# at-cg/PHI

Measured on AMD Instinct MI355X. Metric: read Gbases/s scored (49-hap MHC graph stand-in synMHC-49); reads resident in HBM, parsing and H2D excluded, higher is better.
Workload: dtype u64

## Files before the change

### phi_amd/build.py

```python
import os
import subprocess
import sys

ROOT = os.path.dirname(os.path.dirname(os.path.abspath(__file__)))
CSRC = os.path.join(ROOT, "phi_amd", "csrc")
HIPCC = os.environ.get("HIPCC", "/opt/rocm/bin/hipcc")
ARCH = "gfx950"

HIP_SOURCES = ["sketch.hip", "sketch_pooled.hip", "sketch_win_fixed.hip", "table.hip", "anchors.hip", "contexts.hip", "dp.hip", "dp_events.hip", "phi_abi.hip", "dev_mem.hip", "read_batches.hip", "text_stream.hip", "text_park.hip", "set_graph.hip", "phi_solve.hip", "solve_dev.hip", "phi_comm.hip", "phi_ipc.hip", "reads_text.hip", "walk_text.hip", "edit.hip", "edit_path.hip", "inflate.hip", "gfa_text.hip", "chop.hip", "vcf.hip", "ladder.hip", "panel.hip", "panel_score.hip", "scan.hip", "bam.hip", "calls.hip"]
HIP_HEADERS = ["phi_dev.h", "phi_kernels.h", "phi_ctx.h", "phi_dp_flags.h", "phi_host_par.h", "phi_wave.h", "dp_steps.h", "solve_host.h", "reads_host.h", "bam_header.h", "sketch_dev.h", "sketch_phases.inc", "sketch_minima.inc", "sketch_rounds.inc", "edit_band.inc", os.path.join("host", "panel_choose.h"), os.path.join("..", "..", "include", "phi_amd.h")]


def _run(cmd, cwd=None):
    print("+", " ".join(cmd), flush=True)
    subprocess.check_call(cmd, cwd=cwd)


def _stale(target, deps):
    if not os.path.exists(target):
        return True
    t = os.path.getmtime(target)
    return any(os.path.getmtime(d) > t for d in deps if os.path.exists(d))


EXTRA_FLAGS = {"sketch_pooled.hip": ["-mllvm", "-disable-machine-licm"]}


def build_device(force=False):
    objdir = os.path.join(ROOT, "build", "obj")
    os.makedirs(objdir, exist_ok=True)
    hdrs = [os.path.join(CSRC, h) for h in HIP_HEADERS]
    objs = []
    for src in HIP_SOURCES:
        s = os.path.join(CSRC, src)
        o = os.path.join(objdir, src.replace(".hip", ".o"))
        if force or _stale(o, [s] + hdrs):
            _run([HIPCC, f"--offload-arch={ARCH}", "-O3", "-std=c++17", "-fPIC", "-Wall", "-Wno-unused-function"]
                 + EXTRA_FLAGS.get(src, []) + ["-c", s, "-o", o])
        objs.append(o)
    lib = os.path.join(ROOT, "phi_amd", "libphi_amd.so")
    if force or _stale(lib, objs):
        tmp = f"{lib}.{os.getpid()}.tmp"
        _run([HIPCC, f"--offload-arch={ARCH}", "-shared", "-fPIC", "-o", tmp] + objs + ["-ldl"])
        os.replace(tmp, lib)
    return lib


def build_host(force=False):
    hostdir = os.path.join(CSRC, "host")
    if not os.path.isdir(hostdir):
        return None
    _run(["make", "-C", hostdir] + (["-B"] if force else []))
    return os.path.join(ROOT, "phi_amd", "libphi_host.so")


def build_all(force=False):
    build_device(force)
    build_host(force)


if __name__ == "__main__":
    build_all(force="--force" in sys.argv)
```

### phi_amd/csrc/phi_abi.hip

```cpp
#include <stdarg.h>
#include <stdio.h>
#include <string.h>
#include <algorithm>
#include <future>
#include "phi_ctx.h"
#include "phi_dev.h"

int phi_fail(phi_ctx *c, int code, const char *fmt, ...)
{
    char buf[512];
    va_list ap;
    va_start(ap, fmt);
    vsnprintf(buf, sizeof buf, fmt, ap);
    va_end(ap);
    if (c) {
        std::lock_guard<std::mutex> g(c->err_mu);
        c->last_error = buf;
    }
    return code;
}

int phi_hip_check(phi_ctx *c, hipError_t e, const char *what)
{
    if (e == hipSuccess) return PHI_OK;
    const int code = (e == hipErrorOutOfMemory) ? PHI_ERR_NOMEM : PHI_ERR_DEVICE;
    return phi_fail(c, code, "%s: %s", what, hipGetErrorString(e));
}

extern "C" {

const char *phi_strerror(int status)
{
    switch (status) {
    case PHI_OK: return "ok";
    case PHI_ERR_INVALID: return "invalid argument";
    case PHI_ERR_NOMEM: return "out of memory";
    case PHI_ERR_DEVICE: return "HIP device error";
    case PHI_ERR_STATE: return "call order violated";
    case PHI_ERR_UNSUPPORTED: return "unsupported input";
    case PHI_ERR_WALK: return "walk does not follow the graph";
    case PHI_ERR_OVERFLOW: return "internal table overflow";
    default: return "unknown status";
    }
}

const char *phi_last_error(const phi_ctx *ctx) { return ctx ? ctx->last_error.c_str() : ""; }

int phi_ctx_create(int device_id, phi_ctx **out)
{
    if (!out) return PHI_ERR_INVALID;
    *out = nullptr;
    PhiStageTimer tm("ctx_create");
    int n_dev = 0;
    if (hipGetDeviceCount(&n_dev) != hipSuccess || n_dev <= 0) return PHI_ERR_DEVICE;
    tm.lap("runtime start (hipInit)");
    if (device_id < 0 || device_id >= n_dev) return PHI_ERR_INVALID;
    if (hipSetDevice(device_id) != hipSuccess) return PHI_ERR_DEVICE;
    phi_ctx *c = new (std::nothrow) phi_ctx();
    if (!c) return PHI_ERR_NOMEM;
    c->device = device_id;
    std::future<hipError_t> aux = std::async(std::launch::async, [c, device_id]() {
        hipError_t e = hipSetDevice(device_id);
        if (e == hipSuccess) e = hipStreamCreateWithFlags(&c->aux_stream, hipStreamNonBlocking);
        if (e != hipSuccess) return e;
        void *d = nullptr;
        std::vector<char> h((size_t)1 << 20, 0);
        if (hipMalloc(&d, h.size()) == hipSuccess) {
            (void)phi_dev_poison(d, h.size());
            (void)hipMemcpyAsync(d, h.data(), h.size(), hipMemcpyHostToDevice, c->aux_stream);
            (void)hipMemcpyAsync(h.data(), d, h.size(), hipMemcpyDeviceToHost, c->aux_stream);
            (void)hipMemcpyAsync(d, h.data(), 64, hipMemcpyHostToDevice, c->aux_stream);
            (void)hipMemcpyAsync(h.data(), d, 64, hipMemcpyDeviceToHost, c->aux_stream);
            (void)hipMemsetAsync(d, 0, 4096, c->aux_stream);
            (void)hipStreamSynchronize(c->aux_stream);
            (void)hipFree(d);
        }
        return hipSuccess;
    });
    auto bail = [&](int code) {
        if (aux.valid()) (void)aux.get();
        if (c->own_stream) (void)hipStreamDestroy(c->own_stream);
        if (c->aux_stream) (void)hipStreamDestroy(c->aux_stream);
        phi_dev_free(c->d_scalars); phi_dev_free(c->d_stripes); phi_dev_free(c->alt.stripes);
        delete c;
        return code;
    };
    if (hipStreamCreateWithFlags(&c->own_stream, hipStreamNonBlocking) != hipSuccess) return bail(PHI_ERR_DEVICE);
    c->stream = c->own_stream;
    tm.lap("stream");
    if (phi_dev_ensure(c, c->d_scalars, S_N * 8) || hipMemsetAsync(c->d_scalars.p, 0, S_N * 8, c->stream) != hipSuccess ||
        phi_dev_ensure(c, c->d_stripes, 2 * STRIPE_BYTES) || hipMemsetAsync(c->d_stripes.p, 0, 2 * STRIPE_BYTES, c->stream) != hipSuccess ||
        phi_dev_ensure(c, c->alt.stripes, 2 * STRIPE_BYTES) || hipMemsetAsync(c->alt.stripes.p, 0, 2 * STRIPE_BYTES, c->stream) != hipSuccess)
        return bail(PHI_ERR_DEVICE);
    if (tm.on && getenv("PHI_TIMING_UNITS")) {
        (void)hipStreamSynchronize(c->stream); tm.lap("  scalars");
        phi_warm_sketch(c->stream); (void)hipStreamSynchronize(c->stream); tm.lap("  code object: sketch");
        phi_warm_table(c->stream); (void)hipStreamSynchronize(c->stream); tm.lap("  code object: table");
        phi_warm_anchors(c->stream); (void)hipStreamSynchronize(c->stream); tm.lap("  code object: anchors");
        phi_warm_contexts(c->stream); (void)hipStreamSynchronize(c->stream); tm.lap("  code object: contexts");
        phi_warm_dp(c->stream); (void)hipStreamSynchronize(c->stream); tm.lap("  code object: dp");
        phi_warm_dp_events(c->stream); (void)hipStreamSynchronize(c->stream); tm.lap("  code object: dp_events");
        phi_warm_solve_dev(c->stream); (void)hipStreamSynchronize(c->stream); tm.lap("  code object: solve_dev");
        phi_warm_reads_text(c->stream); (void)hipStreamSynchronize(c->stream); tm.lap("  code object: reads_text");
        phi_warm_scan(c->stream); (void)hipStreamSynchronize(c->stream); tm.lap("  code object: scan");
    }
    phi_warm_sketch(c->stream); phi_warm_table(c->stream); phi_warm_anchors(c->stream); phi_warm_contexts(c->stream);
    phi_warm_dp(c->stream); phi_warm_dp_events(c->stream); phi_warm_solve_dev(c->stream); phi_warm_reads_text(c->stream);
    phi_warm_walk_text(c->stream); phi_warm_scan(c->stream);
    if (hipStreamSynchronize(c->stream) != hipSuccess) return bail(PHI_ERR_DEVICE);
    tm.lap("scalars + code objects");
    if (aux.get() != hipSuccess) { c->aux_stream = nullptr; return bail(PHI_ERR_DEVICE); }
    c->last_error.clear();
    tm.lap("wait for the second stream + first host copies");
    *out = c;
    return PHI_OK;
}

void phi_ctx_destroy(phi_ctx *c)
{
    if (c && c->pin_future.valid()) c->pin_future.wait();
    if (c && c->dp_alloc_future.valid()) (void)c->dp_alloc_future.get();
    if (c && c->h_pin) { (void)hipSetDevice(c->device); (void)hipHostFree(c->h_pin); c->h_pin = nullptr; }
    if (c) { (void)hipSetDevice(c->device); stage_release(c); }
    if (!c) return;
    (void)phi_comm_destroy(c);
    (void)phi_ipc_destroy(c);
    (void)hipSetDevice(c->device);
    (void)hipStreamSynchronize(c->stream);
    phi_ladder_drop(c);
    DevBuf *all[] = {&c->d_anchors, &c->d_cov_all, &c->d_cov_w, &c->d_slots, &c->d_slots2, &c->d_segs, &c->d_ctr, &c->d_vmax, &c->d_lane_walk, &c->d_walk_lane, &c->d_coff, &c->d_blk_ncls, &c->d_rownew, &c->d_blk_bad, &c->d_seg_lo, &c->d_seg_row, &c->d_seg_S, &c->wtext.d_text, &c->panel.d_full, &c->scout.d_scores, &c->d_sel_off, &c->d_sel_tri, &c->d_blk_lo, &c->d_blk_ev, &c->d_blk_S, &c->d_row_out, &c->d_rowend, &c->d_blk_keys, &c->d_blk_carry, &c->d_cov, &c->d_cov2, &c->d_stepdiff, &c->alt.hit, &c->hit_extra[0], &c->hit_extra[1], &c->alt.stripes, &c->spset.d_sp_cnt, &c->rlog.d_novlog, &c->rlog.d_novcnt, &c->rlog.d_ovlist, &c->d_vlen, &c->d_ent_cls, &c->d_cls_rep, &c->d_cls_left, &c->d_cls_mult, &c->d_cls_base, &c->d_cls_rec_off, &c->d_rec_cls, &c->d_rec_rel, &c->d_u_replist, &c->d_adj_off, &c->d_adj, &c->d_topo_rank, &c->d_cnt_edge, &c->d_walk_err, &c->d_sa_cnt, &c->d_sa_cur, &c->d_sa_off, &c->d_sa_idx, &c->d_seq, &c->d_seq_off, &c->d_walk_vtx, &c->d_walk_off, &c->d_topo, &c->d_in_off,
                     &c->d_in_src, &c->d_e_out, &c->d_st_rec, &c->d_st_mask, &c->d_in_packed, &c->d_word, &c->d_wwords, &c->d_wbad,
                     &c->d_wascii, &c->d_wstarts, &c->d_rec_hash, &c->d_rec_pos, &c->d_rec_slot,
                     &c->d_rec_e0, &c->d_rec_e1, &c->d_u_keys, &c->d_u_rep, &c->d_u_uid, &c->d_rt, &c->d_in_s, &c->d_last_walk, &c->d_rowdiag, &c->d_wpre, &c->d_hit, &c->spset.d_sp_keys, &c->d_rbases,
                     &c->d_roff, &c->rlog.d_roff_made, &c->d_peer_send, &c->spset.d_export, &c->d_scalars, &c->d_stripes, &c->d_blk_cnt,
                     &c->d_blk_off, &c->d_flags, &c->d_flags2, &c->d_list, &c->d_list2, &c->d_list3, &c->d_walk_last, &c->d_m_rec, &c->d_m_group,
                     &c->d_g_keys, &c->d_g_rep, &c->d_g_cnt, &c->d_slot_maxcnt, &c->d_slot_multi, &c->d_a_e1,
                     &c->d_g_off, &c->d_g_span, &c->d_a_weight, &c->d_dmax, &c->d_bstart, &c->d_k_rec, &c->d_k_in, &c->d_cvtx, &c->d_ev_e, &c->d_ev_off, &c->d_ev,
                     &c->d_off_end, &c->d_off_start, &c->d_scan_blk, &c->d_scan_blk64, &c->d_scan_blkoff, &c->d_top,
                     &c->d_ent};
    phi_pool_flush(c->device);
    phi_pool_bypass(true);
    struct Bypass { ~Bypass() { phi_pool_bypass(false); } } bypass_guard;
    for (DevBuf *b : all) phi_dev_free(*b);
    for (auto &pr : c->prof_events) { (void)hipEventDestroy(pr.first); (void)hipEventDestroy(pr.second); }
    if (c->h_err) (void)hipHostFree(c->h_err);
    {
        auto &T = c->text;
        for (int i = 0; i < 2; i++) { phi_dev_free(T.text[i]); phi_dev_free(T.bases[i]); phi_dev_free(T.roff[i]); }
        phi_dev_free(T.tile_cnt); phi_dev_free(T.ls); phi_dev_free(T.pre); phi_dev_free(T.blk); phi_dev_free(T.sum);
        if (T.h_sum) (void)hipHostFree(T.h_sum);
        if (T.ev_copy) (void)hipEventDestroy(T.ev_copy);
    }
    phi_bam_drop(c);
    (void)hipStreamDestroy(c->own_stream);
    (void)hipStreamDestroy(c->aux_stream);
    delete c;
}

int phi_set_stream(phi_ctx *c, void *hip_stream)
{
    if (!c) return PHI_ERR_INVALID;
    HIPCHK(hipStreamSynchronize(c->stream));
    c->stream = hip_stream ? (hipStream_t)hip_stream : c->own_stream;
    return PHI_OK;
}

int phi_set_params(phi_ctx *c, int32_t k, int32_t w, float threshold, int32_t recombination, uint32_t flags)
{
    if (!c) return PHI_ERR_INVALID;
    if (c->have_graph) return phi_fail(c, PHI_ERR_STATE, "phi_set_params must precede phi_set_graph");
    if (k < 1 || k > PHI_MAX_K) return phi_fail(c, PHI_ERR_INVALID, "k=%d outside [1,%d]", k, PHI_MAX_K);
    if (w < 1 || w > PHI_MAX_W) return phi_fail(c, PHI_ERR_INVALID, "w=%d outside [1,%d]", w, PHI_MAX_W);
    if (recombination < 0) return phi_fail(c, PHI_ERR_INVALID, "recombination penalty must be >= 0");
    c->k = k; c->w = w; c->threshold = threshold; c->recombination = recombination; c->flags = flags;
    return PHI_OK;
}

}

int sketch_records(phi_ctx *c, const uint64_t *words, const unsigned long long *starts, int64_t n_bases,
                   int32_t k, int32_t w, const uint8_t *ascii_if_bad, DevBuf &out_hash, DevBuf &out_pos,
                   int64_t *n_out)
{
    *n_out = 0;
    const int64_t nb = phi_sketch_num_blocks(n_bases);
    if (nb == 0) return PHI_OK;
    PHICHK(phi_dev_ensure(c, c->d_blk_cnt, (size_t)nb * 4));
    PHICHK(phi_dev_ensure(c, c->d_blk_off, (size_t)(nb + 1) * 8));
    PhiSketchArgs A{};
    A.words = words; A.starts = starts; A.n_bases = n_bases; A.k = k; A.w = w;
    A.ascii = ascii_if_bad; A.allslow = ascii_if_bad ? 1 : 0; A.badbits = nullptr;
    A.block_cnt = c->d_blk_cnt.as<int32_t>();
    A.err = (uint32_t *)scalar(c, S_ERR);
    if (A.allslow) phi_launch_sketch_bytes(c->stream, PHI_MODE_COUNT, A, nullptr);
    else phi_launch_sketch(c->stream, PHI_MODE_COUNT, A);
    PHICHK(phi_scan(c, c->d_blk_cnt.as<int32_t>(), nb, c->d_blk_off.as<int64_t>()));
    int64_t total = 0;
    HIPCHK(hipMemcpyAsync(&total, c->d_blk_off.as<int64_t>() + nb, 8, hipMemcpyDeviceToHost, c->stream));
    HIPCHK(hipStreamSynchronize(c->stream));
    PHICHK(phi_dev_ensure(c, out_hash, (size_t)std::max<int64_t>(total, 1) * 8));
    PHICHK(phi_dev_ensure(c, out_pos, (size_t)std::max<int64_t>(total, 1) * 8));
    A.block_off = c->d_blk_off.as<int64_t>();
    A.out_hash = out_hash.as<uint64_t>();
    A.out_pos = out_pos.as<int64_t>();
    if (A.allslow) phi_launch_sketch_bytes(c->stream, PHI_MODE_WRITE, A, nullptr);
    else phi_launch_sketch(c->stream, PHI_MODE_WRITE, A);
    HIPCHK(hipGetLastError());
    *n_out = total;
    return PHI_OK;
}

extern "C" {

int phi_set_solve_budget(phi_ctx *c, int64_t max_dp_runs)
{
    if (!c) return PHI_ERR_INVALID;
    c->solve_budget = max_dp_runs > 0x7FFFFFFF ? 0x7FFFFFFF : max_dp_runs;
    c->solved = false;
    return PHI_OK;
}

int phi_solve(phi_ctx *c, phi_result *out)
{
    if (!c || !out) return PHI_ERR_INVALID;
    if (!c->have_graph) return phi_fail(c, PHI_ERR_STATE, "phi_solve before phi_set_graph");
    PHICHK(phi_refuse_scout(c, "phi_solve"));
    HIPCHK(hipSetDevice(c->device));
    const int rc = phi_solve_impl(c);
    phi_pool_flush(c->device);
    if (rc) return rc;
    *out = c->result;
    return PHI_OK;
}

int phi_path_sequence(phi_ctx *c, char *buf, int64_t cap)
{
    if (!c || (!buf && cap > 0)) return PHI_ERR_INVALID;
    PHICHK(phi_refuse_scout(c, "phi_path_sequence"));
    if (!c->solved) return phi_fail(c, PHI_ERR_STATE, "phi_path_sequence before phi_solve");
    if (cap < c->result.hap_len) return phi_fail(c, PHI_ERR_INVALID, "buffer too small: need %lld bytes", (long long)c->result.hap_len);
    const int64_t np = (int64_t)c->h_path_vtx.size();
    std::vector<int64_t> at((size_t)np + 1, 0);
    for (int64_t i = 0; i < np; i++) { const int32_t v = c->h_path_vtx[(size_t)i]; at[(size_t)i + 1] = at[(size_t)i] + (c->h_seq_off[v + 1] - c->h_seq_off[v]); }
    phi_parallel_chunks(np, 1 << 15, [&](int64_t lo, int64_t hi, int) {
        for (int64_t i = lo; i < hi; i++) {
            const int32_t v = c->h_path_vtx[(size_t)i];
            memcpy(buf + at[(size_t)i], c->h_seq.data() + c->h_seq_off[v], (size_t)(at[(size_t)i + 1] - at[(size_t)i]));
        }
    });
    return PHI_OK;
}

int phi_sketch(phi_ctx *c, const char *bases, const int64_t *seq_off, int64_t n_seq, int32_t k, int32_t w,
               uint64_t *out_hash, int64_t *out_pos, int32_t *out_seq, int64_t cap, int64_t *n_out)
{
    if (!c || !n_out || n_seq < 0 || (n_seq > 0 && !seq_off)) return PHI_ERR_INVALID;
    if (k < 1 || k > PHI_MAX_K || w < 1 || w > PHI_MAX_W) return phi_fail(c, PHI_ERR_INVALID, "k or w out of range");
    *n_out = 0;
    if (n_seq == 0) return PHI_OK;
    for (int64_t r = 0; r < n_seq; r++)
        if (seq_off[r + 1] < seq_off[r]) return phi_fail(c, PHI_ERR_INVALID, "seq_off not monotone");
    const int64_t n_bases = seq_off[n_seq] - seq_off[0];
    if (n_bases == 0) return PHI_OK;
    if (!bases) return PHI_ERR_INVALID;
    HIPCHK(hipSetDevice(c->device));
    HIPCHK(hipStreamSynchronize(c->stream));
    DevBuf dB, dO, dW, dS, dH, dP;
    int rc = PHI_OK;
    std::vector<int64_t> off(seq_off, seq_off + n_seq + 1);
    for (auto &o : off) o -= seq_off[0];
    do {
        if ((rc = phi_dev_ensure(c, dB, (size_t)n_bases + 64))) break;
        if ((rc = phi_dev_ensure(c, dO, (size_t)(n_seq + 1) * 8))) break;
        const int64_t n_words = (n_bases + 31) / 32;
        if ((rc = phi_dev_ensure(c, dW, (size_t)(n_words + 2) * 8))) break;
        const size_t n_sw = (size_t)(n_bases / 64 + 2);
        if ((rc = phi_dev_ensure(c, dS, n_sw * 8))) break;
        if ((rc = phi_hip_check(c, hipMemcpyAsync(dB.p, bases + seq_off[0], (size_t)n_bases, hipMemcpyHostToDevice, c->stream), "H2D bases"))) break;
        if ((rc = phi_hip_check(c, hipMemcpyAsync(dO.p, off.data(), (size_t)(n_seq + 1) * 8, hipMemcpyHostToDevice, c->stream), "H2D offsets"))) break;
        if ((rc = phi_hip_check(c, hipMemsetAsync(dW.as<uint64_t>() + n_words, 0, 16, c->stream), "memset"))) break;
        if ((rc = phi_hip_check(c, hipMemsetAsync(dS.p, 0, n_sw * 8, c->stream), "memset"))) break;
        if ((rc = phi_hip_check(c, hipMemsetAsync(scalar(c, S_NBAD), 0, 8, c->stream), "memset"))) break;
        phi_launch_mark_starts(c->stream, dO.as<int64_t>(), n_seq, dS.as<unsigned long long>());
        phi_launch_pack_ascii(c->stream, dB.as<uint8_t>(), n_bases, dW.as<uint64_t>(), n_words, nullptr,
                              (unsigned long long *)scalar(c, S_NBAD));
        if ((rc = phi_hip_check(c, hipStreamSynchronize(c->stream), "sync"))) break;
// ... 210 lines not shown
```

### phi_amd/csrc/phi_ctx.h

```cpp
#pragma once
#include <stdint.h>
#include <stdarg.h>
#include <stdio.h>
#include <stdlib.h>
#include <algorithm>
#include <atomic>
#include <chrono>
#include <future>
#include <mutex>
#include <string>
#include <thread>
#include <vector>
#include <hip/hip_runtime.h>
#include "../../include/phi_amd.h"
#include "phi_kernels.h"
#include "phi_host_par.h"
#include "solve_host.h"
#include "reads_host.h"

struct DevBuf {
    void *p = nullptr;
    size_t cap = 0;
    uint32_t gen = 0;
    template <class T> T *as() const { return reinterpret_cast<T *>(p); }
};

template <class T> struct PhiRawBuf {
    T *p = nullptr;
    size_t n = 0;
    PhiRawBuf() = default;
    PhiRawBuf(const PhiRawBuf &) = delete;
    PhiRawBuf &operator=(const PhiRawBuf &) = delete;
    ~PhiRawBuf() { free(p); }
    bool resize(size_t m)
    {
        free(p);
        p = m ? static_cast<T *>(malloc(m * sizeof(T))) : nullptr;
        n = p ? m : 0;
        return m == 0 || p != nullptr;
    }
    size_t size() const { return n; }
    T *data() const { return p; }
    T &operator[](size_t i) const { return p[i]; }
};

struct PhiComm;
struct PhiIpc;
#define PHI_HIT_RING 4
struct PhiPeers;

struct phi_ctx {
    int device = 0;
    PhiComm *comm = nullptr;
    PhiPeers *peers = nullptr;
    int peer_rank = 0;
    PhiIpc *ipc = nullptr;
    hipStream_t own_stream = nullptr, stream = nullptr;
    hipStream_t aux_stream = nullptr;
    std::string last_error;
    std::mutex err_mu;

    int32_t k = 31, w = 25, recombination = 100;
    float threshold = 1.0f;
    uint32_t flags = PHI_FLAG_QCLP | PHI_FLAG_MIXED;
    int64_t solve_budget = 4096;

    bool have_graph = false;
    int32_t n_vtx = 0, n_walks = 0;
    std::vector<char> h_seq;
    std::vector<int64_t> h_seq_off, h_adj_off, h_walk_off, h_walk_base;
    std::vector<int32_t> h_adj, h_topo_rank, h_topo;
    PhiRawBuf<int32_t> h_walk_vtx;
    int64_t n_entries = 0, walk_bases = 0;

#define WT_TILE 4096
    struct PhiWalkText {
        bool ready = false;
        int32_t n_walks = 0;
        std::vector<int64_t> tile0, t_len;
        std::vector<int32_t> ends;
        DevBuf d_text;
    } wtext;
    bool walks_on_device = false;
    int64_t walks_on_device_n = 0;
    struct PhiChop {
        bool on = false;
        std::vector<int32_t> first;
        phi_chop_info info{};
    } chop;
    struct PhiPanel {
        bool on = false;
        std::vector<int32_t> origin;
        std::vector<int32_t> kept;
        phi_panel_info info{};
        DevBuf d_full;
        std::vector<int64_t> full_off;
    } panel;
    struct PhiScout {
        bool on = false;
        DevBuf d_scores;
        int32_t n_blocks = 0;
    } scout;
    struct PhiVcf {
        bool have = false;
        phi_vcf_info info{};
    } vcf;

    DevBuf d_seq, d_seq_off, d_walk_vtx, d_walk_off, d_topo, d_in_off, d_in_src;
    DevBuf d_e_out, d_st_rec, d_st_mask, d_in_packed;
    int dp_nw = 1;
    DevBuf d_wwords, d_wstarts, d_wbad, d_wascii;
    DevBuf d_vlen;
    DevBuf d_ent_cls;
    DevBuf d_cls_rep, d_cls_left, d_cls_mult, d_cls_base, d_cls_rec_off;
    int64_t n_cls = 0, cls_bases = 0;
    double index_gpu_ms = 0.0;
    DevBuf d_rec_hash, d_rec_pos, d_rec_cls, d_rec_rel, d_rec_slot, d_rec_e0, d_rec_e1;
    int64_t n_rec = 0;
    DevBuf d_u_keys, d_u_rep, d_u_uid, d_u_replist;
    DevBuf d_rt;
    uint64_t rt_buckets = 0, rt_mask = 0;
    void *h_stage[2] = {nullptr, nullptr};
    hipEvent_t stage_ev[2] = {nullptr, nullptr};
    DevBuf d_wpre;
    DevBuf d_rowdiag;
    DevBuf d_in_s, d_last_walk;
    int64_t n_unique = 0;
    uint64_t u_cap = 0;
    DevBuf d_hit;
    DevBuf hit_extra[PHI_HIT_RING - 2];
    int hit_n = 2, hit_idx = 0;

    struct PhiSpectrumSet {
        DevBuf d_sp_keys;
        uint64_t sp_cap = 0;
        DevBuf d_sp_cnt;
        DevBuf d_export;
        int64_t sp_set_gen = -1;
        int64_t sp_gen = 0;
        void new_generation() { sp_gen++; }
        void new_graph() { sp_set_gen = -1; }
    } spset;
    struct PhiReadLog {
        DevBuf d_novlog, d_novcnt;
        int32_t nov_shift = 6;
        int64_t log_chunks = 0, log_done = 0;
        int64_t logged_done = 0;
        int64_t last_log_chunks = 0;
        DevBuf d_ovlist;
        int64_t ov_cap = 0, ov_done = 0, ov_bound = 0;
        bool async_batches = false;
        bool next_flag_zeroed = false;
        DevBuf d_roff_made;
        void flushed() { log_chunks = log_done = 0; ov_done = 0; ov_bound = 0; }
        void new_generation() { flushed(); logged_done = 0; last_log_chunks = 0; next_flag_zeroed = false; }
    } rlog;
    int64_t reads_bases = 0, reads_count = 0;
    int64_t spectrum_override = -1;
    DevBuf d_rbases, d_roff, d_peer_send;
    DevBuf d_scalars;
    DevBuf d_stripes;
    struct PhiReadBufs {
        DevBuf hit, stripes;
        bool needs_clean = false;
    } alt;

    uint32_t *h_err = nullptr;
    struct PhiTextStream {
        bool active = false, irregular = false, started = false, detached = false;
        bool carry_stale = false;
        int mode = 0;
        int64_t fed = 0, taken = 0;
        uint32_t carry_cap = 0, chunk_cap = 0, line_cap = 0;
        DevBuf text[2], bases[2], roff[2], tile_cnt, ls, pre, blk, sum;
        int slot = 0;
        uint32_t carry_len = 0, carry_at = 0;
        std::vector<char> h_carry;
        PhiTextSummary *h_sum = nullptr;
        hipEvent_t ev_copy = nullptr;
        int last_slot = -1;
        int64_t last_reads = 0, last_bases = 0;
        bool last_uniform = false;
        int dbg_slot = 0;
        int64_t dbg_reads = 0, dbg_bases = 0;
        uint32_t why = 0, first_bad = 0;
    } text;

    struct PhiBamStream {
        bool active = false, failed = false, header_done = false;
        int32_t n_ref = 0;
        uint32_t tile = 0, list_cap = 0, max_tiles = 0, max_rec = 0;
        uint32_t carry_cap = 0, chunk_cap = 0;
        std::vector<unsigned char> h_hdr;
        int64_t fed = 0;
        DevBuf text[2];
        DevBuf bases, roff, sum;
        DevBuf t_first, t_exit, t_status, t_cnt, t_skip, t_list, t_has, t_has_pre, t_use, t_base;
        DevBuf rec_pos, rec_keep, kidx, klen, kseq, krev;
        int slot = 0;
        uint32_t carry_len = 0, carry_at = 0;
        void *h_sum = nullptr;
        hipEvent_t ev_copy = nullptr;
        int64_t one_len = -1;
        int64_t dbg_reads = 0, dbg_bases = 0;
        phi_bam_info info{};
    } bam;

    struct PhiLadder {
        bool collecting = false, have_store = false, have_plan = false;
        int64_t first_ordinal = 0;
        int64_t n_reads = 0, n_bases = 0;
        int64_t one_len = -1;
        DevBuf d_bases, d_off;
        DevBuf d_pbases, d_poff, d_pidx, d_psrc, d_wg, d_tab;
        int64_t band_read0[PHI_LADDER_MAX_LEVELS + 1] = {0}, band_pos[PHI_LADDER_MAX_LEVELS + 1] = {0};
        int32_t scored = 0;
        phi_ladder_info info{};
    } ladder;

    DevBuf d_blk_cnt, d_blk_off, d_flags, d_flags2, d_list, d_list2, d_list3, d_walk_last;
    DevBuf d_sel_off, d_sel_tri;
    DevBuf d_adj_off, d_adj, d_topo_rank, d_cnt_edge, d_walk_err;
    DevBuf d_sa_cnt, d_sa_cur, d_sa_off, d_sa_idx;

    DevBuf d_m_rec, d_m_group, d_g_keys, d_g_rep, d_g_cnt, d_slot_maxcnt, d_slot_multi;
    DevBuf d_a_e1, d_g_off, d_g_span, d_a_weight;
    DevBuf d_dmax, d_bstart, d_top, d_ent, d_word;
    bool dp_dense_ready = false;
    bool dp_events = false;
    int32_t n_k = 0;
    int64_t n_ev = 0;
    std::vector<int32_t> h_cstep, h_kstep;
    std::vector<int32_t> h_k_cut_ok;
    bool dp_blocks = false;
    int32_t n_blk = 0, blk_ring = 1024, blk_max_len = 0;
    std::vector<int32_t> h_blk_lo;
    DevBuf d_blk_lo, d_blk_ev, d_blk_S, d_row_out, d_rowend, d_blk_keys, d_blk_carry, d_cov, d_cov2, d_stepdiff;
    bool dp_cls = false;
    int32_t blk_cls_target = 16;
    bool blk_no_small = false;
    int32_t blk_ls = 64;
    DevBuf d_lane_walk, d_walk_lane, d_coff, d_blk_ncls, d_rownew, d_blk_bad;
    DevBuf d_seg_lo, d_seg_row, d_seg_S;
    DevBuf d_k_rec, d_k_in, d_cvtx, d_ev_e, d_ev_off, d_ev, d_off_end, d_off_start, d_scan_blk, d_scan_blk64, d_scan_blkoff;
    DevBuf d_anchors, d_cov_all, d_cov_w, d_slots, d_slots2, d_segs, d_ctr, d_vmax;
    int64_t n_kept = 0, n_dp = 0;
    bool anchors_host = false;
    PhiAnchorSpan h_kept, h_dp;
    std::vector<PhiAnchorHost> h_dp_own;
    void *h_pin = nullptr;
    size_t h_pin_cap = 0;
    std::future<void> pin_future;
    std::future<int> dp_alloc_future;
    std::vector<uint64_t> h_kept_hash;
    std::vector<int32_t> h_path_vtx, h_path_hap;
    std::vector<int64_t> h_n_minimizers, h_n_anchors;
    phi_result result{};
    bool solved = false;
    struct PhiPathSeg { int32_t h; int64_t es, ee; };
    std::vector<PhiPathSeg> path_segs;
    struct PhiCalls {
        bool have = false;
        std::vector<int64_t> pos, ref_off, alt_off;
        std::vector<int32_t> anchor;
        std::vector<char> ref_bytes, alt_bytes;
        int64_t span[4] = {0, 0, 0, 0};
        phi_calls_info info{};
    } calls;

    bool prof = false;
    std::vector<std::pair<hipEvent_t, hipEvent_t>> prof_events;
    int prof_period = 1;
    uint64_t prof_seq = 0;
    size_t prof_used = 0;
// ... 103 lines not shown
```

### phi_amd/csrc/phi_dev.h

```cpp
#pragma once
#include <stdint.h>

#if defined(__HIPCC__)
#include <hip/hip_runtime.h>
#define PHI_HD __host__ __device__ __forceinline__
#else
#define PHI_HD static inline
#endif

#define PHI_EMPTY_KEY 0xFFFFFFFFFFFFFFFFull

PHI_HD uint32_t phi_code(uint32_t c) { return ((c >> 1) ^ (c >> 2)) & 3u; }
PHI_HD bool phi_is_acgt(uint32_t c)
{
    c &= 0xDFu;
    return c == 'A' || c == 'C' || c == 'G' || c == 'T';
}

PHI_HD uint64_t phi_extract64(const uint64_t *words, int64_t i)
{
    const int64_t wi = i >> 5;
    const int s = (int)(i & 31) * 2;
    const uint64_t hi = words[wi];
    if (s == 0) return hi;
// ... 17 lines not shown
        hi = q;
        for (int64_t step = 1;; step <<= 1) {
            if (hi - step <= 0) break;
            if (off[hi - step] <= g) { lo = hi - step; break; }
            hi -= step;
        }
    }
    while (hi - lo > 1) {
        const int64_t mid = (lo + hi) >> 1;
        if (off[mid] <= g) lo = mid; else hi = mid;
    }
    return lo;
}

PHI_HD uint64_t phi_kmask(int k) { return k >= 32 ? ~0ull : ((1ull << (2 * k)) - 1); }

PHI_HD uint64_t phi_revcomp(uint64_t f, int k)
{
    uint64_t x = ~f;
    x = ((x >> 2) & 0x3333333333333333ull) | ((x & 0x3333333333333333ull) << 2);
    x = ((x >> 4) & 0x0F0F0F0F0F0F0F0Full) | ((x & 0x0F0F0F0F0F0F0F0Full) << 4);
    x = __builtin_bswap64(x);
    return x >> (64 - 2 * k);
}

PHI_HD uint64_t phi_rotl64(uint64_t x, int r) { return (x << r) | (x >> (64 - r)); }

PHI_HD uint64_t phi_mul64(uint64_t a, uint64_t c)
{
#if defined(__HIP_DEVICE_COMPILE__)
    const uint32_t alo = (uint32_t)a, ahi = (uint32_t)(a >> 32), clo = (uint32_t)c, chi = (uint32_t)(c >> 32);
    const uint64_t t = (uint64_t)alo * clo;
    uint32_t lo = (uint32_t)t, hi = (uint32_t)(t >> 32) + alo * chi + ahi * clo;
    asm("" : "+v"(lo), "+v"(hi));
    return ((uint64_t)hi << 32) | lo;
#else
    return a * c;
#endif
}

PHI_HD uint64_t phi_x5_plus(uint64_t h, uint64_t c)
{
#if defined(__HIP_DEVICE_COMPILE__)
    uint64_t q = h << 2;
    asm("" : "+v"(q));
    return q + h + c;
#else
    return h * 5 + c;
#endif
}

PHI_HD uint64_t phi_fmix64(uint64_t k)
{
    k ^= k >> 33; k = phi_mul64(k, 0xff51afd7ed558ccdull);
    k ^= k >> 33; k = phi_mul64(k, 0xc4ceb9fe1a85ec53ull);
    k ^= k >> 33;
    return k;
}

PHI_HD uint32_t phi_ascii4(uint32_t x)
{
#if defined(__HIP_DEVICE_COMPILE__)
    uint32_t t = __umul24(x, 0x100401u);
    asm("" : "+v"(t));
#else
    uint32_t t = x | (x << 10);
    t = t | (x << 20);
#endif
    const uint32_t sel = ((t << 4) | (x >> 6)) & 0x03030303u;
#if defined(__HIP_DEVICE_COMPILE__)
    return __builtin_amdgcn_perm(0x54474341u, 0x54474341u, sel);
#else
    uint32_t r = 0;
    for (int j = 0; j < 4; j++) r |= ((0x54474341u >> (8 * ((sel >> (8 * j)) & 3))) & 0xFFu) << (8 * j);
    return r;
#endif
}

PHI_HD uint64_t phi_ascii8(uint32_t x16)
{
    return (uint64_t)phi_ascii4((x16 >> 8) & 0xFFu) | ((uint64_t)phi_ascii4(x16 & 0xFFu) << 32);
}

PHI_HD uint64_t phi_murmur_lanes(uint64_t e0, uint64_t e1, uint64_t e2, uint64_t e3, int k)
{
    const uint64_t c1 = 0x87c37b91114253d5ull, c2 = 0x4cf5ad432745937full;
    uint64_t h1 = 0, h2 = 0;
    const int nblocks = k >> 4;
    uint64_t t1, t2;
    if (nblocks >= 1) {
        uint64_t k1 = e0, k2 = e1;
        k1 = phi_mul64(k1, c1); k1 = phi_rotl64(k1, 31); k1 = phi_mul64(k1, c2); h1 ^= k1;
        h1 = phi_rotl64(h1, 27); h1 += h2; h1 = phi_x5_plus(h1, 0x52dce729);
        k2 = phi_mul64(k2, c2); k2 = phi_rotl64(k2, 33); k2 = phi_mul64(k2, c1); h2 ^= k2;
        h2 = phi_rotl64(h2, 31); h2 += h1; h2 = phi_x5_plus(h2, 0x38495ab5);
        t1 = e2; t2 = e3;
    } else {
        t1 = e0; t2 = e1;
    }
    if (nblocks == 2) {
        uint64_t k1 = t1, k2 = t2;
        k1 = phi_mul64(k1, c1); k1 = phi_rotl64(k1, 31); k1 = phi_mul64(k1, c2); h1 ^= k1;
        h1 = phi_rotl64(h1, 27); h1 += h2; h1 = phi_x5_plus(h1, 0x52dce729);
        k2 = phi_mul64(k2, c2); k2 = phi_rotl64(k2, 33); k2 = phi_mul64(k2, c1); h2 ^= k2;
        h2 = phi_rotl64(h2, 31); h2 += h1; h2 = phi_x5_plus(h2, 0x38495ab5);
    } else {
        const int rem = k & 15;
        if (rem > 8) { uint64_t k2 = t2; k2 = phi_mul64(k2, c2); k2 = phi_rotl64(k2, 33); k2 = phi_mul64(k2, c1); h2 ^= k2; }
        if (rem > 0) { uint64_t k1 = t1; k1 = phi_mul64(k1, c1); k1 = phi_rotl64(k1, 31); k1 = phi_mul64(k1, c2); h1 ^= k1; }
    }
    h1 ^= (uint64_t)k; h2 ^= (uint64_t)k;
    h1 += h2; h2 += h1;
    h1 = phi_fmix64(h1); h2 = phi_fmix64(h2);
    h1 += h2; h2 += h1;
    return h1 ^ h2;
}

PHI_HD uint64_t phi_murmur_lanes8(const uint64_t *e, int k)
{
    const uint64_t c1 = 0x87c37b91114253d5ull, c2 = 0x4cf5ad432745937full;
    uint64_t h1 = 0, h2 = 0;
    const int nblocks = k >> 4;
    for (int b = 0; b < nblocks; b++) {
        uint64_t k1 = e[2 * b], k2 = e[2 * b + 1];
        k1 = phi_mul64(k1, c1); k1 = phi_rotl64(k1, 31); k1 = phi_mul64(k1, c2); h1 ^= k1;
        h1 = phi_rotl64(h1, 27); h1 += h2; h1 = phi_x5_plus(h1, 0x52dce729);
        k2 = phi_mul64(k2, c2); k2 = phi_rotl64(k2, 33); k2 = phi_mul64(k2, c1); h2 ^= k2;
        h2 = phi_rotl64(h2, 31); h2 += h1; h2 = phi_x5_plus(h2, 0x38495ab5);
    }
    const int rem = k & 15;
    if (rem > 8) { uint64_t k2 = e[2 * nblocks + 1]; k2 = phi_mul64(k2, c2); k2 = phi_rotl64(k2, 33); k2 = phi_mul64(k2, c1); h2 ^= k2; }
    if (rem > 0) { uint64_t k1 = e[2 * nblocks]; k1 = phi_mul64(k1, c1); k1 = phi_rotl64(k1, 31); k1 = phi_mul64(k1, c2); h1 ^= k1; }
    h1 ^= (uint64_t)k; h2 ^= (uint64_t)k;
    h1 += h2; h2 += h1;
    h1 = phi_fmix64(h1); h2 = phi_fmix64(h2);
    h1 += h2; h2 += h1;
    return h1 ^ h2;
}

PHI_HD uint64_t phi_kmer_hash(uint64_t val, int k)
{
    const uint64_t L = val << (64 - 2 * k);
    uint64_t e[4];
#pragma unroll
    for (int g = 0; g < 4; g++) {
        uint64_t a = phi_ascii8((uint32_t)(L >> (48 - 16 * g)) & 0xFFFFu);
        const int nb = k - 8 * g;
        if (nb <= 0) a = 0;
        else if (nb < 8) a &= (1ull << (8 * nb)) - 1;
        e[g] = a;
    }
    return phi_murmur_lanes(e[0], e[1], e[2], e[3], k);
}
```

### phi_amd/csrc/phi_kernels.h

```cpp
#pragma once
#include <stdint.h>
#include <hip/hip_runtime.h>
#include "phi_dp_flags.h"

#ifndef PHI_TPB
#define PHI_TPB 256

#endif
#define PHI_WCH 512
#define PHI_MAX_W 256
#define PHI_MAX_K 64
#define PHI_MAX_K_PACKED 32
#define PHI_MAX_PROBE 4096
#define PHI_RT_OVERFLOWED 1u
static inline int phi_nov_shift(int w)
{
    const int want = (3 * 2 * PHI_WCH) / (2 * (w + 1));
    int sh = 4;
    while ((1 << sh) < want && sh < 9) sh++;
    return sh;
}
#define PHI_STRIPES 256

typedef uint32_t phi_ent_t;
#define PHI_MAX_ENTRIES (((int64_t)1 << 32) - 64)

enum { PHI_MODE_COUNT = 0, PHI_MODE_WRITE = 1, PHI_MODE_PROBE = 2 };

#define PHI_MB_ERR 8
#define PHI_MB_SCORED 16
#define PHI_MB_GATHERED 17
#define PHI_MB_BLOCKS 18

#define PHI_KERR_SENTINEL 1u
#define PHI_KERR_TABLE_FULL 2u
#define PHI_KERR_WALK_EDGE 4u
#define PHI_KERR_CSR_ID 32u
#define PHI_KERR_DP_QUEUE 16u
#define PHI_KERR_DP_CLASSES 64u

struct PhiSketchArgs {
    const uint64_t *words;
    const unsigned long long *starts;
    int64_t n_bases;
    int32_t k, w;
    const unsigned long long *badbits;
    const uint8_t *ascii;
    int32_t allslow;
    int32_t *block_cnt;
    const int64_t *block_off;
    uint64_t *out_hash;
    int64_t *out_pos;
    unsigned long long *n_logged;
    unsigned long long *n_emitted;
    const uint64_t *u_rt; uint64_t u_bmask;
    uint8_t *hit;
    uint32_t *err;
    uint64_t *nov_log; uint16_t *nov_cnt; int64_t log_base; int32_t nov_shift;
    uint64_t *ov_list; unsigned long long *ov_count; int64_t ov_cap;
    const int64_t *read_off; int64_t n_reads;
    uint32_t reads_per_base_q32;
    int32_t uniform_len;
    double inv_len;
    uint32_t inv_len_q32;
    int32_t wave_stride;
    int32_t q_clean;
    int32_t win_reads;
    unsigned long long *ov_zero;
    unsigned long long *ipc_mb; unsigned long long ipc_scored, ipc_need;
    uint64_t *q_hit_words; int64_t q_n_hit_words; uint64_t *q_stripes; int64_t q_n_stripe_words;
};

void phi_launch_pack_ascii(hipStream_t st, const uint8_t *bases, int64_t n, uint64_t *words, int64_t n_words,
                           uint32_t *badbits, unsigned long long *n_bad);
void phi_launch_mark_starts(hipStream_t st, const int64_t *seq_off, int64_t n_seq, unsigned long long *starts);

void phi_launch_sketch_bytes(hipStream_t st, int mode, const PhiSketchArgs &A, const unsigned long long *batch_bad);
void phi_launch_reset_reads(hipStream_t st, uint64_t *hit_words, int64_t n_hit_words, uint64_t *stripes, int64_t n_stripe_words);
int64_t phi_sketch_num_blocks(int64_t n_bases);
int phi_sketch_win_reads(int k, int w, int64_t uniform_len, int64_t n_reads, int64_t n_bases);
int64_t phi_sketch_read_chunks(int k, int w, int64_t uniform_len, int64_t n_reads, int64_t n_bases);
void phi_launch_sketch(hipStream_t st, int mode, const PhiSketchArgs &A, hipEvent_t t0 = nullptr, hipEvent_t t1 = nullptr);

void phi_launch_table_build(hipStream_t st, const uint64_t *rec_hash, int64_t n_rec, uint64_t *u_keys,
                            uint32_t *u_rep, uint64_t u_mask, uint32_t *rec_slot, uint32_t *err);
void phi_launch_rep_flags(hipStream_t st, const uint32_t *rec_slot, int64_t n_rec, const uint32_t *u_rep,
                          uint8_t *flags);
void phi_launch_table_compact(hipStream_t st, const int32_t *rep_list, int64_t n_unique, const uint64_t *rec_hash, int64_t n_rec,
                              uint64_t *keys, uint32_t *uid, uint64_t mask, uint32_t *rec_slot, uint32_t *err);
void phi_launch_share_hist(hipStream_t st, const uint64_t *keys, int64_t cap, const int32_t *n_walks_of, unsigned long long *hist);
void phi_launch_slot_uid(hipStream_t st, const int32_t *rep_list, int64_t n_unique, const uint32_t *rec_slot,
                         uint32_t *u_uid);
void phi_launch_read_table(hipStream_t st, const uint64_t *keys, const uint32_t *uid, int64_t cap, uint64_t *rt,
                           int64_t n_buckets, uint32_t *err);
void phi_launch_fill_u64(hipStream_t st, uint64_t *p, int64_t n, uint64_t v);
void phi_launch_fill_u32(hipStream_t st, uint32_t *p, int64_t n, uint32_t v);
void phi_launch_iota_i64(hipStream_t st, int64_t *p, int64_t n, int64_t step);
void phi_launch_spectrum_insert(hipStream_t st, const uint64_t *hashes, int64_t n, uint64_t *sp_keys,
                                uint64_t sp_mask, unsigned long long *sp_count, const uint64_t *u_keys, uint64_t u_mask,
                                const uint32_t *u_uid, uint8_t *hit, uint32_t *err);
void phi_launch_spectrum_flush(hipStream_t st, const uint64_t *nov_log, const uint16_t *nov_cnt, int64_t c_lo, int64_t c_hi, int32_t shift,
                               uint64_t *sp_keys, uint64_t sp_mask, unsigned long long *sp_count, uint32_t *err);
void phi_launch_count_flags(hipStream_t st, const uint8_t *flags, int64_t n, unsigned long long *n_out);
void phi_launch_spectrum_export(hipStream_t st, const uint64_t *sp_keys, int64_t cap, uint64_t *out,
                                unsigned long long *n_out);

struct PhiClassArgs {
    const int32_t *walk_vtx; const int64_t *walk_off; int32_t n_walks; int64_t n_entries;
    const int32_t *vlen; const uint8_t *seq; const int64_t *seq_off;
    int32_t tail_need;
    uint64_t seed;
    uint64_t *t_keys; uint32_t *t_rep; uint32_t *t_mult; uint64_t t_mask;
    uint32_t *ent_slot;
    uint32_t *err;
};
struct PhiExpandArgs {
    const int32_t *ent_cls; int64_t e_lo, e_hi;
    const int32_t *cls_rec_off; const phi_ent_t *cls_rep;
    const uint8_t *sel; const int32_t *sel_cnt;
    int32_t *block_cnt; const int64_t *block_off;
    const uint64_t *rec_hash; const int32_t *rec_rel; const int64_t *ent_base; uint64_t *out_hash; int64_t *out_pos;
    const uint32_t *rec_slot; const uint32_t *u_uid; const phi_ent_t *rec_e0; const phi_ent_t *rec_e1; uint32_t *out_tri;
};
void phi_launch_vlen(hipStream_t st, const int64_t *seq_off, int64_t n_vtx, int32_t *vlen);
void phi_launch_walk_bases(hipStream_t st, const int32_t *walk_vtx, const int32_t *vlen, const int64_t *walk_off, int32_t n_walks,
                           int64_t n_entries, unsigned long long *out);
void phi_launch_walk_rec_counts(hipStream_t st, const int32_t *ent_cls, const int32_t *cls_rec_off, const int64_t *walk_off,
                                int32_t n_walks, int64_t n_entries, unsigned long long *out);
void phi_launch_class_insert(hipStream_t st, const PhiClassArgs &A);
void phi_launch_class_verify(hipStream_t st, const PhiClassArgs &A, uint8_t *is_rep);
void phi_launch_class_ids(hipStream_t st, const phi_ent_t *cls_rep, int64_t n_cls, const uint32_t *ent_slot, int64_t n_entries,
                          const uint32_t *t_mult, uint32_t *t_cid, int32_t *cls_mult, int32_t *ent_cls);
void phi_launch_class_len(hipStream_t st, const PhiClassArgs &A, const phi_ent_t *cls_rep, int64_t n_cls, int32_t *cls_len, uint8_t *cls_left);
void phi_launch_pack_classes(hipStream_t st, const uint8_t *seq, const int64_t *seq_off, const int32_t *walk_vtx, const int32_t *vlen,
                             const phi_ent_t *cls_rep, const uint8_t *cls_left, const int64_t *cls_base, int64_t n_cls, uint64_t *words,
                             int64_t n_words, uint32_t *badbits, uint8_t *ascii, unsigned long long *n_bad);
void phi_launch_class_rec(hipStream_t st, const int64_t *raw_pos, int64_t n_raw, const int64_t *cls_base, int64_t n_cls,
                          const phi_ent_t *cls_rep, const uint8_t *cls_left, const int32_t *walk_vtx, const int32_t *vlen, int32_t k,
                          uint8_t *keep, int32_t *r_cls, int32_t *r_rel, phi_ent_t *r_e0, phi_ent_t *r_e1);
void phi_launch_class_rec_gather(hipStream_t st, const int32_t *idx, int64_t n, const uint64_t *raw_hash, const int32_t *r_cls,
                                 const int32_t *r_rel, const phi_ent_t *r_e0, const phi_ent_t *r_e1, uint64_t *o_hash, int32_t *o_cls,
                                 int32_t *o_rel, phi_ent_t *o_e0, phi_ent_t *o_e1);
void phi_launch_class_rec_off(hipStream_t st, const int32_t *rec_cls, int64_t n_rec, int64_t n_cls, int32_t *off);
int64_t phi_expand_num_blocks(int64_t n_entries);
void phi_launch_expand_count(hipStream_t st, const PhiExpandArgs &A);
void phi_launch_expand_write(hipStream_t st, const PhiExpandArgs &A, int kind);
void phi_launch_class_sel_count(hipStream_t st, const uint8_t *sel, const int32_t *cls_rec_off, int64_t n_cls, int32_t *sel_cnt);
void phi_launch_class_sel_tri(hipStream_t st, const uint8_t *sel, const int32_t *cls_rec_off, int64_t n_cls, const int32_t *sel_off, const phi_ent_t *cls_rep,
                              const uint32_t *rec_slot, const uint32_t *u_uid, const phi_ent_t *rec_e0, const phi_ent_t *rec_e1, int32_t *sel_tri);
void phi_launch_expand_tri(hipStream_t st, const int32_t *ent_cls, int64_t e_lo, int64_t e_hi, const int32_t *sel_off, const int32_t *sel_tri,
                           const int64_t *block_off, uint32_t *out_tri, phi_ent_t *a_e1, uint8_t *a_span, const int64_t *walk_off, int32_t n_walks,
                           unsigned long long *walk_cnt, unsigned long long *prep, int64_t n_anchors);
void phi_launch_mark_list(hipStream_t st, const int32_t *list, const int32_t *through, int64_t n, uint8_t *sel);
void phi_launch_share_count_cls(hipStream_t st, const int32_t *ent_cls, int64_t e_lo, int64_t e_hi, const int32_t *cls_rec_off,
                                const uint32_t *rec_slot, int32_t walk, int32_t *last_walk, int32_t *n_walks_of);
void phi_launch_entry_len_range(hipStream_t st, const int32_t *walk_vtx, const int32_t *vlen, int64_t e_lo, int64_t n, int32_t *lens);

#define PHI_KERR_FP_COLLISION 8u
void phi_launch_walk_edges(hipStream_t st, const int32_t *walk_vtx, const int64_t *walk_off, int32_t n_walks, int64_t n_entries, int32_t n_vtx,
                           const int64_t *adj_off, const int32_t *adj, const int64_t *seq_off, const int32_t *topo_rank,
                           uint8_t *e_out, int32_t *cnt_edge, unsigned long long *st_mask, int32_t nw64, int32_t *err);
void phi_launch_csr_count(hipStream_t st, const uint32_t *triples, int64_t n, int64_t n_ids, int32_t *cnt, uint32_t *err);
void phi_launch_csr_scatter(hipStream_t st, const uint32_t *triples, int64_t n, int64_t n_ids, const int32_t *off, int32_t *cur,
                            int32_t *idx);
void phi_launch_csr_sort(hipStream_t st, const int32_t *off, int64_t n_ids, int32_t *idx);
void phi_launch_match_flags(hipStream_t st, const uint32_t *rec_slot, int64_t n_rec, const uint32_t *u_uid,
                            const uint8_t *hit, uint8_t *flags);

struct PhiFilterArgs {
    const uint32_t *rec_slot; const phi_ent_t *rec_e0; const phi_ent_t *rec_e1;
    const int32_t *walk_vtx;
    const int32_t *rec_cls; const int32_t *cls_mult;
    const int32_t *m_rec;
    uint64_t *g_keys; int32_t *g_rep; uint32_t *g_cnt; uint64_t g_mask; uint64_t seed;
    int32_t *m_group;
    const uint32_t *u_uid;
    uint32_t *slot_maxcnt;
    uint8_t *slot_multi;
    float limit;
    unsigned long long *counters;
    uint32_t *err;
};
void phi_launch_group_insert(hipStream_t st, const PhiFilterArgs &A, int64_t n_matched);
void phi_launch_group_count(hipStream_t st, const PhiFilterArgs &A, int64_t n_matched);
void phi_launch_group_max(hipStream_t st, const PhiFilterArgs &A, int64_t n_matched);
void phi_launch_slot_count(hipStream_t st, const PhiFilterArgs &A, int64_t u_cap);
void phi_launch_kept_flags(hipStream_t st, const PhiFilterArgs &A, int64_t n_matched, uint8_t *kept, uint8_t *dp);
void phi_launch_gather_i32(hipStream_t st, const int32_t *src, const uint32_t *idx, int64_t n, int32_t *out);
void phi_launch_gather_u64(hipStream_t st, const uint64_t *src, const int32_t *idx, int64_t n, uint64_t *out);
void phi_launch_entry_csr(hipStream_t st, const phi_ent_t *a_e1, int64_t n_a, int64_t n_entries, int64_t *g_off);

#define PHI_DP_CHUNK 128
#define PHI_DP_RING 2048
#define PHI_SCOUT_MAX_WALKS 65535
#define PHI_DP_MAX_WALKS 1022

struct PhiDpArgs {
    int32_t n_vtx, n_walks;
    const int32_t *st_rec;
    const unsigned long long *st_mask;
    const int32_t *in_packed;
    const int64_t *walk_off;
    const uint64_t *word;
    const int64_t *g_off; const uint8_t *g_span; const uint8_t *a_weight;
    int32_t cost;
    int32_t *dmax;
    int32_t *bstart;
    int32_t *tops;
    int32_t *ent_src, *ent_h;
};
void phi_launch_dp(hipStream_t st, const PhiDpArgs &A);

#define PHI_DP_EVENT_MAX_WALKS 256
#define PHI_DP_EVENT_SAFE_WALKS 128
struct PhiDpEventArgs {
    int32_t n_k, n_walks;
    int64_t n_ev;
    const int32_t *k_rec;
    const int32_t *k_in_packed;
    const int64_t *walk_off;
    const phi_ent_t *ev_e;
    const int64_t *ev_off;
    void *ev;
    const int64_t *g_off; const uint8_t *g_span; const uint8_t *a_weight;
    int32_t cost;
    int32_t *dmax, *bstart;
    int32_t *tops;
    int32_t *ent_src, *ent_h;
    uint32_t *err;
    int32_t q_limit;
    int32_t n_blk, blk_ring;
    int32_t blk_max_len;
    int32_t lane_stride;
    const int32_t *lane_walk;
    int32_t *rownew_out;
    int32_t *rowdiag_out;
    const int32_t *blk_lo;
    const int32_t *blk_ev;
    const int32_t *blk_S;
    int32_t *row_out; int32_t *rowend_out;
    int32_t *blk_keys_out; int32_t *blk_carry;
};
void phi_launch_dp_events(hipStream_t st, const PhiDpEventArgs &A);
void phi_launch_dp_block_rows(hipStream_t st, const PhiDpEventArgs &A);
void phi_launch_dp_block_paths(hipStream_t st, const PhiDpEventArgs &A);
void phi_launch_anchor_prep(hipStream_t st, const uint32_t *tri, int64_t n, const int64_t *walk_off, int32_t n_walks, phi_ent_t *a_e1, uint8_t *a_span,
                            unsigned long long *walk_cnt, unsigned long long *out);
void phi_launch_vertex_most(hipStream_t st, const int64_t *g_off, int64_t n_entries, const int32_t *walk_vtx, int32_t *vmax);
void phi_launch_sum_i32(hipStream_t st, const int32_t *v, int64_t n, unsigned long long *out);
void phi_launch_repeat_walk(hipStream_t st, const uint32_t *tri, int64_t lo, int64_t hi, int32_t walk, int32_t *last, uint8_t *flags);
void phi_launch_weights(hipStream_t st, const uint32_t *tri, int64_t n, const uint8_t *in_s, uint8_t *wgt);
void phi_launch_path_cover(hipStream_t st, bool clear, const phi_ent_t *segs, int32_t n_seg, const int64_t *g_off, const uint32_t *tri, const uint8_t *wgt,
                           int32_t *cov_all, int32_t *cov_w, unsigned long long *ctr, uint32_t *twice, int64_t twice_cap);
void phi_launch_uncovered_slots(hipStream_t st, const uint32_t *slots, int64_t n, const int32_t *cov_all, unsigned long long *ctr, uint32_t *out);
struct PhiBlkClassArgs {
// ... 88 lines not shown
```

### phi_amd/csrc/read_batches.hip

```cpp
#include <string.h>
#include "phi_ctx.h"
#include "phi_dev.h"

static unsigned long long *logged_stripes(phi_ctx *c) { return c->d_stripes.as<unsigned long long>(); }
static unsigned long long *emit_stripes(phi_ctx *c) { return c->d_stripes.as<unsigned long long>() + PHI_STRIPES * 8; }

int phi_flush_reset(phi_ctx *c) { return c && c->ipc ? phi_ipc_wait_pending(c) : PHI_OK; }

static void swap_read_bufs(phi_ctx *c)
{
    if (c->hit_n == PHI_HIT_RING) {
        const DevBuf old = c->d_hit;
        c->d_hit = c->alt.hit; c->alt.hit = c->hit_extra[0]; c->hit_extra[0] = c->hit_extra[1]; c->hit_extra[1] = old;
        c->hit_idx = (c->hit_idx + 1) % PHI_HIT_RING;
    } else {
        std::swap(c->d_hit, c->alt.hit);
    }
    std::swap(c->d_stripes, c->alt.stripes);
}

static int sum_stripes(phi_ctx *c, const void *d, int n_sets, uint64_t *out)
{
    std::vector<uint64_t> h((size_t)n_sets * PHI_STRIPES * 8);
    int rc = phi_hip_check(c, phi_copy_sync(c, h.data(), d, (size_t)n_sets * STRIPE_BYTES, hipMemcpyDeviceToHost), "D2H counters");
    if (rc) return rc;
    for (int s_ = 0; s_ < n_sets; s_++) {
        uint64_t a = 0;
        for (int i = 0; i < PHI_STRIPES; i++) a += h[((size_t)s_ * PHI_STRIPES + i) * 8];
        out[s_] = a;
    }
    return PHI_OK;
}

int phi_read_counts(phi_ctx *c, uint64_t *n_logged, uint64_t *n_emitted)
{
    int frc = phi_flush_reset(c);
    if (frc) return frc;
    if (hipStreamSynchronize(c->stream) != hipSuccess) return phi_fail(c, PHI_ERR_DEVICE, "stream synchronize failed");
    uint64_t v[2];
    int rc = sum_stripes(c, c->d_stripes.p, 2, v);
    if (rc) return rc;
    if (n_logged) *n_logged = v[0];
    if (n_emitted) *n_emitted = v[1];
    return PHI_OK;
}

static int sp_set_size(phi_ctx *c, uint64_t *n)
{
    auto &S = c->spset;
    *n = 0;
    if (S.sp_cap == 0 || S.sp_set_gen != S.sp_gen) return PHI_OK;
    return sum_stripes(c, S.d_sp_cnt.p, 1, n);
}

static int sp_clear(phi_ctx *c, uint64_t cap)
{
    auto &S = c->spset;
    if (cap != S.sp_cap || !S.d_sp_keys.p) {
        phi_dev_free(S.d_sp_keys);
        S.sp_cap = 0;
        PHICHK(phi_dev_ensure(c, S.d_sp_keys, cap * 8));
        S.sp_cap = cap;
    }
    PHICHK(phi_dev_ensure(c, S.d_sp_cnt, STRIPE_BYTES));
    phi_launch_fill_u64(c->stream, S.d_sp_keys.as<uint64_t>(), (int64_t)cap, PHI_EMPTY_KEY);
    HIPCHK(hipMemsetAsync(S.d_sp_cnt.p, 0, STRIPE_BYTES, c->stream));
    return PHI_OK;
}

static int sp_reserve(phi_ctx *c, uint64_t in_set, uint64_t more)
{
    auto &S = c->spset;
    const uint64_t need = phi_set_capacity(in_set, more);
    if (S.sp_set_gen != S.sp_gen) {
        PHICHK(sp_clear(c, phi_set_reusable(S.sp_cap, need) ? S.sp_cap : need));
        S.sp_set_gen = S.sp_gen;
        return PHI_OK;
    }
    if (need <= S.sp_cap) return PHI_OK;
    PHICHK(phi_dev_ensure(c, S.d_export, (size_t)std::max<uint64_t>(in_set, 1) * 8));
    HIPCHK(hipMemsetAsync(scalar(c, S_EXPORT), 0, 8, c->stream));
    phi_launch_spectrum_export(c->stream, S.d_sp_keys.as<uint64_t>(), (int64_t)S.sp_cap, S.d_export.as<uint64_t>(),
                               (unsigned long long *)scalar(c, S_EXPORT));
    HIPCHK(hipStreamSynchronize(c->stream));
    PHICHK(sp_clear(c, need));
    phi_launch_spectrum_insert(c->stream, S.d_export.as<uint64_t>(), (int64_t)in_set, S.d_sp_keys.as<uint64_t>(), S.sp_cap - 1,
                               S.d_sp_cnt.as<unsigned long long>(), nullptr, 0, nullptr, nullptr, (uint32_t *)scalar(c, S_ERR));
    return PHI_OK;
}

int phi_sp_flush(phi_ctx *c, uint64_t *n_in_set)
{
    auto &S = c->spset;
    auto &L = c->rlog;
    PHICHK(phi_sync_check(c));
    L.async_batches = false;
    uint64_t logged = 0, in_set = 0;
    PHICHK(phi_read_counts(c, &logged, nullptr));
    unsigned long long ov_now = 0;
    HIPCHK(phi_copy_sync(c, &ov_now, scalar(c, S_OVCNT + (int)(S.sp_gen % 3)), 8, hipMemcpyDeviceToHost));
    if ((int64_t)ov_now > L.ov_cap) ov_now = (unsigned long long)L.ov_cap;
    const bool pending = L.log_chunks > L.log_done || (int64_t)ov_now > L.ov_done;
    PHICHK(sp_set_size(c, &in_set));
    if (pending) {
        const uint64_t more = logged > (uint64_t)L.logged_done ? logged - (uint64_t)L.logged_done : 0;
        PHICHK(sp_reserve(c, in_set, more));
        if (L.log_chunks > L.log_done)
            phi_launch_spectrum_flush(c->stream, L.d_novlog.as<uint64_t>(), L.d_novcnt.as<uint16_t>(), L.log_done, L.log_chunks, L.nov_shift,
                                      S.d_sp_keys.as<uint64_t>(), S.sp_cap - 1, S.d_sp_cnt.as<unsigned long long>(), (uint32_t *)scalar(c, S_ERR));
        if ((int64_t)ov_now > L.ov_done)
            phi_launch_spectrum_insert(c->stream, L.d_ovlist.as<uint64_t>() + L.ov_done, (int64_t)ov_now - L.ov_done, S.d_sp_keys.as<uint64_t>(),
                                       S.sp_cap - 1, S.d_sp_cnt.as<unsigned long long>(), nullptr, 0, nullptr, nullptr, (uint32_t *)scalar(c, S_ERR));
        HIPCHK(hipGetLastError());
        L.log_done = L.log_chunks; L.ov_done = (int64_t)ov_now; L.logged_done = (int64_t)logged;
        PHICHK(phi_sync_check(c));
        PHICHK(sp_set_size(c, &in_set));
    }
    if (n_in_set) *n_in_set = in_set;
    return PHI_OK;
}

int phi_spectrum_count(phi_ctx *c, uint64_t *n_distinct)
{
    uint64_t in_set = 0, flagged = 0;
    PHICHK(phi_sp_flush(c, &in_set));
    if (c->n_unique > 0) {
        HIPCHK(hipMemsetAsync(scalar(c, S_EXPORT), 0, 8, c->stream));
        phi_launch_count_flags(c->stream, c->d_hit.as<uint8_t>(), c->n_unique, (unsigned long long *)scalar(c, S_EXPORT));
        HIPCHK(hipMemcpyAsync(&flagged, scalar(c, S_EXPORT), 8, hipMemcpyDeviceToHost, c->stream));
        HIPCHK(hipStreamSynchronize(c->stream));
    }
    *n_distinct = in_set + flagged;
    return PHI_OK;
}

int phi_sync_check(phi_ctx *c)
{
    PHICHK(phi_flush_reset(c));
    HIPCHK(hipStreamSynchronize(c->stream));
    uint64_t s[S_N];
    HIPCHK(phi_copy_sync(c, s, c->d_scalars.p, sizeof s, hipMemcpyDeviceToHost));
    const uint32_t err = (uint32_t)s[S_ERR];
    if (err & PHI_KERR_TABLE_FULL) return phi_fail(c, PHI_ERR_OVERFLOW, "open-addressed table overflow (probe bound %d), or the overflow list of novel read hashes ran full under a batch handed over with phi_add_reads_device", PHI_MAX_PROBE);
    if (err & PHI_KERR_SENTINEL) return phi_fail(c, PHI_ERR_UNSUPPORTED, "a minimiser hashes to UINT64_MAX (table sentinel)");
    return PHI_OK;
}

extern "C" {

int phi_add_reads_device(phi_ctx *c, const void *d_bases, const void *d_read_off, int64_t n_reads, int64_t n_bases)
{
    const int rc = phi_add_reads_device_impl(c, d_bases, d_read_off, n_reads, n_bases, false);
    if (c && rc == PHI_OK) c->rlog.async_batches = true;
    return rc;
}

}

int phi_add_reads_device_impl(phi_ctx *c, const void *d_bases, const void *d_read_off, int64_t n_reads, int64_t n_bases, bool replay)
{
    if (!c) return PHI_ERR_INVALID;
    if (!c->have_graph) return phi_fail(c, PHI_ERR_STATE, "phi_add_reads before phi_set_graph");
    if (n_reads < 0 || n_bases < 0 || (n_bases > 0 && !d_bases)) return phi_fail(c, PHI_ERR_INVALID, "phi_add_reads: bad arguments");
    if (__builtin_expect(c->ladder.collecting, 0)) return phi_ladder_collect(c, d_bases, d_read_off, n_reads, n_bases);
    auto &L = c->rlog;
    int64_t uniform_len = 0;
    if (!d_read_off && n_reads > 0 && n_bases > 0) {
        if (n_bases % n_reads) return phi_fail(c, PHI_ERR_INVALID, "phi_add_reads_device without offsets: %lld bases are not %lld reads of one length", (long long)n_bases, (long long)n_reads);
        const PhiOneLength one = phi_device_one_length(n_reads, n_bases);
        if (one.make_offsets) {
            PHICHK(phi_dev_ensure(c, L.d_roff_made, (size_t)(n_reads + 1) * 8));
            phi_launch_iota_i64(c->stream, L.d_roff_made.as<int64_t>(), n_reads + 1, one.step);
            d_read_off = L.d_roff_made.p;
        }
        uniform_len = one.uniform_len;
    }
    if (n_reads == 0 || n_bases == 0) { if (!replay) c->reads_count += n_reads; return PHI_OK; }
    HIPCHK(hipSetDevice(c->device));
    c->solved = false;
    const int64_t n_log_chunks = phi_sketch_read_chunks(c->k, c->w, uniform_len, n_reads, n_bases);
    {
        size_t budget = (size_t)1 << 30;
        if (const char *e = getenv("PHI_NOVLOG_BUDGET")) budget = (size_t)std::max<long long>(atoll(e), 1);
        const PhiLogPlan P = phi_log_plan(L.log_chunks, L.last_log_chunks, replay, n_log_chunks, L.nov_shift, L.d_novlog.cap, L.d_novcnt.cap, budget);
        L.log_chunks = P.base;
        if (P.flush_first) {
            PHICHK(phi_sp_flush(c, nullptr));
            L.flushed();
            HIPCHK(hipMemsetAsync(scalar(c, S_OVCNT + (int)(c->spset.sp_gen % 3)), 0, 8, c->stream));
        }
        if (P.log_bytes) {
            PHICHK(phi_dev_grow_keep(c, L.d_novlog, P.log_bytes, P.keep_log));
            PHICHK(phi_dev_grow_keep(c, L.d_novcnt, P.cnt_bytes, P.keep_cnt));
        }
        if (!replay) {
            L.ov_bound += phi_ov_batch_bound(n_bases, c->w);
            const char *e = getenv("PHI_OVLIST_CAP");
            if (e && !L.d_ovlist.p) {
                L.ov_cap = std::max<long long>(atoll(e), 1);
                PHICHK(phi_dev_ensure(c, L.d_ovlist, (size_t)L.ov_cap * 8));
            } else if (const int64_t cap = phi_ov_capacity(L.ov_bound, L.ov_cap); !e && cap != L.ov_cap) {
                PHICHK(phi_dev_grow_keep(c, L.d_ovlist, (size_t)cap * 8, (size_t)L.ov_cap * 8));
                L.ov_cap = cap;
            }
        }
    }
    PhiSketchArgs A{};
    A.ascii = (const uint8_t *)d_bases;
    A.read_off = (const int64_t *)d_read_off; A.n_reads = n_reads;
    A.uniform_len = (int32_t)uniform_len; A.inv_len = uniform_len ? 1.0 / (double)uniform_len : 0.0;
    A.inv_len_q32 = phi_inv_len_q32(uniform_len); A.reads_per_base_q32 = phi_reads_per_base_q32(n_reads, n_bases);
    A.allslow = c->k > PHI_MAX_K_PACKED;
    A.n_bases = n_bases; A.k = c->k; A.w = c->w;
    A.n_logged = replay ? nullptr : logged_stripes(c);
    A.n_emitted = replay ? nullptr : emit_stripes(c);
    A.u_rt = c->d_rt.as<uint64_t>(); A.u_bmask = c->rt_mask;
    A.hit = c->d_hit.as<uint8_t>();
    A.err = (uint32_t *)scalar(c, S_ERR);
    A.nov_log = L.d_novlog.as<uint64_t>(); A.nov_cnt = L.d_novcnt.as<uint16_t>(); A.log_base = L.log_chunks; A.nov_shift = L.nov_shift;
    A.ov_list = L.d_ovlist.as<uint64_t>(); A.ov_cap = L.ov_cap;
    A.ov_count = (unsigned long long *)scalar(c, S_OVCNT + (int)(c->spset.sp_gen % 3));
    L.log_chunks += n_log_chunks; L.last_log_chunks = n_log_chunks;
    if (c->alt.needs_clean) {
        A.q_clean = 1;
        A.ov_zero = (unsigned long long *)scalar(c, S_OVCNT + (int)((c->spset.sp_gen + 1) % 3));
        A.q_hit_words = c->alt.hit.as<uint64_t>(); A.q_n_hit_words = c->n_unique / 8 + 1;
        A.q_stripes = c->alt.stripes.as<uint64_t>(); A.q_n_stripe_words = 2 * PHI_STRIPES * 8;
        c->alt.needs_clean = false;
        L.next_flag_zeroed = true;
    }
    phi_ipc_launch_args(c, A);
    hipEvent_t t0 = nullptr, t1 = nullptr;
    if (c->prof && c->prof_period > 0 && (c->prof_seq++ % c->prof_period) == 0) {
        if (c->prof_used == c->prof_events.size()) {
            hipEvent_t a, b;
            HIPCHK(hipEventCreate(&a));
            HIPCHK(hipEventCreate(&b));
            c->prof_events.emplace_back(a, b);
        }
        t0 = c->prof_events[c->prof_used].first; t1 = c->prof_events[c->prof_used].second;
        c->prof_used++;
        c->prof_bases += n_bases;
    }
    phi_launch_sketch(c->stream, PHI_MODE_PROBE, A, t0, t1);
    HIPCHK(hipGetLastError());
    if (!replay) { c->reads_bases += n_bases; c->reads_count += n_reads; }
    return PHI_OK;
}


int replay_if_full(phi_ctx *c, uint32_t err, const void *d_bases, const void *d_off, int64_t n_reads, int64_t n_bases)
{
    for (int attempt = 0; attempt < 8 && (err & PHI_KERR_TABLE_FULL); attempt++) {
        unsigned long long *cnt = (unsigned long long *)scalar(c, S_OVCNT + (int)(c->spset.sp_gen % 3));
        unsigned long long wanted = 0;
        HIPCHK(phi_copy_sync(c, &wanted, cnt, 8, hipMemcpyDeviceToHost));
        const PhiOvReplay R = phi_ov_replay(wanted, c->rlog.ov_cap);
        PHICHK(phi_dev_grow_keep(c, c->rlog.d_ovlist, (size_t)R.cap * 8, (size_t)R.valid * 8));
        c->rlog.ov_cap = R.cap;
        HIPCHK(phi_copy_sync(c, cnt, &R.valid, 8, hipMemcpyHostToDevice));
        err &= ~PHI_KERR_TABLE_FULL;
        HIPCHK(phi_copy_sync(c, scalar(c, S_ERR), &err, 4, hipMemcpyHostToDevice));
        PHICHK(phi_add_reads_device_impl(c, d_bases, d_off, n_reads, n_bases, true));
        HIPCHK(phi_copy_sync(c, &err, scalar(c, S_ERR), 4, hipMemcpyDeviceToHost));
    }
    return PHI_OK;
}

static int score_wait_replay(phi_ctx *c, const void *d_bases, const void *d_read_off, int64_t n_reads, int64_t n_bases, PhiStageTimer *tm)
{
    PHICHK(phi_add_reads_device_impl(c, d_bases, d_read_off, n_reads, n_bases, false));
    HIPCHK(hipMemcpyAsync(c->h_err, scalar(c, S_ERR), 4, hipMemcpyDeviceToHost, c->stream));
    HIPCHK(hipStreamSynchronize(c->stream));
    if (tm) tm->lap("H2D + sketch + probe");
    if (*c->h_err & PHI_KERR_TABLE_FULL) {
        PHICHK(replay_if_full(c, *c->h_err, d_bases, d_read_off, n_reads, n_bases));
        if (tm) tm->lap("overflow list grown, batch replayed");
    }
    return PHI_OK;
}

int phi_score_resident_batch(phi_ctx *c, const void *d_bases, const void *d_read_off, int64_t n_reads, int64_t n_bases)
{
    if (c->rlog.async_batches) { PHICHK(phi_sync_check(c)); c->rlog.async_batches = false; }
    if (!c->h_err) HIPCHK(hipHostMalloc((void **)&c->h_err, 64, hipHostMallocDefault));
    return score_wait_replay(c, d_bases, d_read_off, n_reads, n_bases, nullptr);
}

extern "C" {

int phi_add_reads(phi_ctx *c, const char *bases, const int64_t *read_off, int64_t n_reads)
{
    if (!c) return PHI_ERR_INVALID;
    if (!c->have_graph) return phi_fail(c, PHI_ERR_STATE, "phi_add_reads before phi_set_graph");
    if (n_reads < 0 || (n_reads > 0 && !read_off)) return phi_fail(c, PHI_ERR_INVALID, "phi_add_reads: bad arguments");
    if (n_reads == 0) return PHI_OK;
    if (read_off[0] != 0) return phi_fail(c, PHI_ERR_INVALID, "read_off must start at 0");
    const int64_t first_bad = phi_offsets_first_bad(read_off, n_reads, false, 0);
    if (first_bad >= 0) return phi_fail(c, PHI_ERR_INVALID, "read_off not monotone at read %lld", (long long)first_bad);
    const int64_t n_bases = read_off[n_reads];
    if (n_bases > 0 && !bases) return phi_fail(c, PHI_ERR_INVALID, "phi_add_reads: bases is null");
    const bool uniform = phi_reads_one_length(read_off, n_reads);
    HIPCHK(hipSetDevice(c->device));
    PhiStageTimer tm("add_reads");
    if (c->rlog.async_batches) { PHICHK(phi_sync_check(c)); c->rlog.async_batches = false; }
    PHICHK(phi_dev_ensure(c, c->d_roff, (size_t)(n_reads + 1) * 8));
    if (!c->h_err) HIPCHK(hipHostMalloc((void **)&c->h_err, 64, hipHostMallocDefault));
    tm.lap("buffers");
    PHICHK(phi_dev_ensure(c, c->d_rbases, (size_t)std::max<int64_t>(n_bases, 1)));
    if (!uniform) HIPCHK(hipMemcpyAsync(c->d_roff.p, read_off, (size_t)(n_reads + 1) * 8, hipMemcpyHostToDevice, c->stream));
    if (n_bases) HIPCHK(hipMemcpyAsync(c->d_rbases.p, bases, (size_t)n_bases, hipMemcpyHostToDevice, c->stream));
    return score_wait_replay(c, c->d_rbases.p, uniform ? nullptr : c->d_roff.p, n_reads, n_bases, &tm);
}

int phi_reset_reads(phi_ctx *c)
{
    if (!c) return PHI_ERR_INVALID;
    if (!c->have_graph) return phi_fail(c, PHI_ERR_STATE, "phi_reset_reads before phi_set_graph");
    HIPCHK(hipSetDevice(c->device));
    const bool front_dirty = c->alt.needs_clean;
    swap_read_bufs(c);
    c->alt.needs_clean = true;
    if (front_dirty) {
        PHICHK(phi_ipc_before_generation(c, c->spset.sp_gen + 1));
        phi_launch_reset_reads(c->stream, c->d_hit.as<uint64_t>(), c->d_hit.p ? c->n_unique / 8 + 1 : 0, c->d_stripes.as<uint64_t>(), 2 * PHI_STRIPES * 8);
        HIPCHK(hipGetLastError());
    }
    c->spset.new_generation();
    if (!c->rlog.next_flag_zeroed) HIPCHK(hipMemsetAsync(scalar(c, S_OVCNT + (int)(c->spset.sp_gen % 3)), 0, 8, c->stream));
    c->rlog.new_generation();
    c->reads_bases = 0; c->reads_count = 0; c->spectrum_override = -1;
    c->solved = false;
    c->ladder.scored = 0;
    return PHI_OK;
}

int phi_reads_stats(phi_ctx *c, int64_t *n_reads, int64_t *n_bases, int64_t *n_emitted, int64_t *n_distinct)
{
    if (!c) return PHI_ERR_INVALID;
    if (!c->have_graph) return phi_fail(c, PHI_ERR_STATE, "phi_reads_stats before phi_set_graph");
    HIPCHK(hipSetDevice(c->device));
    PHICHK(phi_sync_check(c));
    uint64_t nd = 0, ne = 0;
    PHICHK(phi_read_counts(c, nullptr, &ne));
    PHICHK(phi_spectrum_count(c, &nd));
    if (n_reads) *n_reads = c->reads_count;
    if (n_bases) *n_bases = c->reads_bases;
    if (n_emitted) *n_emitted = (int64_t)ne;
    if (n_distinct) *n_distinct = (int64_t)nd;
    return PHI_OK;
}

int phi_hits_buffer(phi_ctx *c, void **d_hits, int64_t *n)
{
    if (!c || !d_hits || !n) return PHI_ERR_INVALID;
    if (!c->have_graph) return phi_fail(c, PHI_ERR_STATE, "phi_hits_buffer before phi_set_graph");
    HIPCHK(hipSetDevice(c->device));
    PHICHK(phi_flush_reset(c));
    *d_hits = c->d_hit.p;
    *n = c->n_unique;
    return PHI_OK;
}

int phi_read_table(phi_ctx *c, void **d_table, int64_t *n_buckets)
{
    if (!c || !d_table || !n_buckets) return PHI_ERR_INVALID;
    if (!c->have_graph) return phi_fail(c, PHI_ERR_STATE, "phi_read_table before phi_set_graph");
    *d_table = c->d_rt.p;
    *n_buckets = (int64_t)c->rt_buckets;
    return PHI_OK;
}
// ... 48 lines not shown
```

### phi_amd/csrc/set_graph.hip

```cpp
#include <string.h>
#include <algorithm>
#include <future>
#include <memory>
#include "phi_ctx.h"
#include "phi_dev.h"
#include "dp_steps.h"

static int build_read_table(phi_ctx *c)
{
    uint64_t nb = pow2_at_least(std::max<uint64_t>(64, (16 * (uint64_t)c->n_unique + 2) / 3));
    if (const char *e = getenv("PHI_READ_TABLE_BUCKETS")) nb = pow2_at_least(std::max<long long>(atoll(e), 1));
    uint32_t err0 = 0;
    HIPCHK(hipMemcpyAsync(&err0, scalar(c, S_ERR), 4, hipMemcpyDeviceToHost, c->stream));
    HIPCHK(hipStreamSynchronize(c->stream));
    for (int attempt = 0;; attempt++) {
        PHICHK(phi_dev_ensure(c, c->d_rt, nb * 32));
        phi_launch_read_table(c->stream, c->d_u_keys.as<uint64_t>(), c->d_u_uid.as<uint32_t>(), (int64_t)c->u_cap,
                              c->d_rt.as<uint64_t>(), (int64_t)nb, (uint32_t *)scalar(c, S_ERR));
        uint32_t err = 0;
        HIPCHK(hipMemcpyAsync(&err, scalar(c, S_ERR), 4, hipMemcpyDeviceToHost, c->stream));
        HIPCHK(hipStreamSynchronize(c->stream));
        if ((err0 & PHI_KERR_TABLE_FULL) || !(err & PHI_KERR_TABLE_FULL)) break;
        if (attempt >= 40) return phi_fail(c, PHI_ERR_OVERFLOW, "read table overflow at %llu buckets (internal error)", (unsigned long long)nb);
        err &= ~PHI_KERR_TABLE_FULL;
        HIPCHK(phi_copy_sync(c, scalar(c, S_ERR), &err, 4, hipMemcpyHostToDevice));
        nb *= 2;
    }
    c->rt_buckets = nb; c->rt_mask = nb - 1;
    return PHI_OK;
}

static int build_classes(phi_ctx *c, int32_t n_vtx, int32_t n_walks, int64_t n_entries)
{
    PhiStageTimer tg("set_graph");
    hipEvent_t ev0 = nullptr, ev1 = nullptr;
    HIPCHK(hipEventCreate(&ev0));
    HIPCHK(hipEventCreate(&ev1));
    struct EvGuard { hipEvent_t a, b; ~EvGuard() { (void)hipEventDestroy(a); (void)hipEventDestroy(b); } } evg{ev0, ev1};
    HIPCHK(hipEventRecord(ev0, c->stream));
    PHICHK(phi_dev_ensure(c, c->d_vlen, (size_t)n_vtx * 4));
    phi_launch_vlen(c->stream, c->d_seq_off.as<int64_t>(), n_vtx, c->d_vlen.as<int32_t>());
    PHICHK(phi_dev_ensure(c, c->d_list, (size_t)(n_walks + 1) * 8));
    HIPCHK(hipMemsetAsync(c->d_list.p, 0, (size_t)(n_walks + 1) * 8, c->stream));
    phi_launch_walk_bases(c->stream, c->d_walk_vtx.as<int32_t>(), c->d_vlen.as<int32_t>(), c->d_walk_off.as<int64_t>(), n_walks, n_entries,
                          c->d_list.as<unsigned long long>());
    c->h_walk_base.assign(n_walks + 1, 0);
    HIPCHK(hipMemcpyAsync(c->h_walk_base.data() + 1, c->d_list.p, (size_t)n_walks * 8, hipMemcpyDeviceToHost, c->stream));

    tg.lap("[gpu thread]     events, vlen, walk bases");
    PHICHK(phi_dev_ensure(c, c->d_ent_cls, (size_t)n_entries * 4));
    PHICHK(phi_dev_ensure(c, c->d_flags, (size_t)n_entries));
    DevBuf t_keys, t_rep, t_mult;
    PhiDevGuard guard{{&t_keys, &t_rep, &t_mult}};
    PhiClassArgs A{};
    A.walk_vtx = c->d_walk_vtx.as<int32_t>(); A.walk_off = c->d_walk_off.as<int64_t>(); A.n_walks = n_walks; A.n_entries = n_entries;
    A.vlen = c->d_vlen.as<int32_t>(); A.seq = c->d_seq.as<uint8_t>(); A.seq_off = c->d_seq_off.as<int64_t>();
    A.tail_need = c->w + c->k - 2;
    A.ent_slot = c->d_ent_cls.as<uint32_t>();
    A.err = (uint32_t *)scalar(c, S_ERR);
    const uint64_t cap_max = pow2_at_least(std::max<uint64_t>(1024, 2 * (uint64_t)n_entries));
    uint64_t cap = std::min(cap_max, pow2_at_least(std::max<uint64_t>(1024, 4 * (uint64_t)n_vtx)));
    tg.lap("[gpu thread]     entry buffers");
    for (int attempt = 0;; attempt++) {
        PHICHK(phi_dev_ensure(c, t_keys, cap * 8));
        PHICHK(phi_dev_ensure(c, t_rep, cap * 4));
        PHICHK(phi_dev_ensure(c, t_mult, cap * 4));
        A.t_keys = t_keys.as<uint64_t>(); A.t_rep = t_rep.as<uint32_t>(); A.t_mult = t_mult.as<uint32_t>(); A.t_mask = cap - 1;
        A.seed = 0x13198A2E03707344ull + 0x9E3779B97F4A7C15ull * (uint64_t)attempt;
        phi_launch_fill_u64(c->stream, A.t_keys, (int64_t)cap, PHI_EMPTY_KEY);
        phi_launch_fill_u32(c->stream, A.t_rep, (int64_t)cap, 0xFFFFFFFFu);
        HIPCHK(hipMemsetAsync(A.t_mult, 0, cap * 4, c->stream));
        phi_launch_class_insert(c->stream, A);
        uint32_t err = 0;
        HIPCHK(hipMemcpyAsync(&err, scalar(c, S_ERR), 4, hipMemcpyDeviceToHost, c->stream));
        HIPCHK(hipStreamSynchronize(c->stream));
        if (err & PHI_KERR_TABLE_FULL) {
            if (cap == cap_max) return phi_fail(c, PHI_ERR_OVERFLOW, "walk-context table overflow (internal error)");
            cap = std::min(cap_max, cap * 8);
            err &= ~PHI_KERR_TABLE_FULL;
            HIPCHK(phi_copy_sync(c, scalar(c, S_ERR), &err, 4, hipMemcpyHostToDevice));
            attempt--;
            continue;
        }
        phi_launch_class_verify(c->stream, A, c->d_flags.as<uint8_t>());
        HIPCHK(hipMemcpyAsync(&err, scalar(c, S_ERR), 4, hipMemcpyDeviceToHost, c->stream));
        HIPCHK(hipStreamSynchronize(c->stream));
        if (!(err & PHI_KERR_FP_COLLISION)) break;
        if (attempt >= 7) return phi_fail(c, PHI_ERR_DEVICE, "walk-context fingerprints collide under 8 seeds (internal error)");
        err &= ~PHI_KERR_FP_COLLISION;
        HIPCHK(phi_copy_sync(c, scalar(c, S_ERR), &err, 4, hipMemcpyHostToDevice));
    }
    tg.lap("[gpu thread]     table insert + verify");
    for (int32_t h = 0; h < n_walks; h++) c->h_walk_base[h + 1] += c->h_walk_base[h];
    c->walk_bases = c->h_walk_base[n_walks];
    PHICHK(phi_compact(c, c->d_flags.as<uint8_t>(), n_entries, c->d_cls_rep, &c->n_cls));
    const int64_t nc = c->n_cls;
    tg.lap("[gpu thread]     compact representatives");
    PHICHK(phi_dev_ensure(c, c->d_cls_mult, (size_t)nc * 4));
    PHICHK(phi_dev_ensure(c, c->d_cls_left, (size_t)nc));
    PHICHK(phi_dev_ensure(c, c->d_cls_base, (size_t)(nc + 1) * 8));
    PHICHK(phi_dev_ensure(c, c->d_cls_rec_off, (size_t)(nc + 1) * 4));
    phi_launch_class_ids(c->stream, c->d_cls_rep.as<phi_ent_t>(), nc, A.ent_slot, n_entries, A.t_mult, A.t_rep, c->d_cls_mult.as<int32_t>(),
                         c->d_ent_cls.as<int32_t>());
    PHICHK(phi_dev_ensure(c, c->d_list3, (size_t)nc * 4));
    phi_launch_class_len(c->stream, A, c->d_cls_rep.as<phi_ent_t>(), nc, c->d_list3.as<int32_t>(), c->d_cls_left.as<uint8_t>());
    PHICHK(phi_scan(c, c->d_list3.as<int32_t>(), nc, c->d_cls_base.as<int64_t>()));
    int64_t run = 0;
    HIPCHK(hipMemcpyAsync(&run, c->d_cls_base.as<int64_t>() + nc, 8, hipMemcpyDeviceToHost, c->stream));
    HIPCHK(hipStreamSynchronize(c->stream));
    c->cls_bases = run;
    if (tg.on) fprintf(stderr, "[phi timing] set_graph: %lld entries in %lld classes, %lld bases of class space for %lld bases of walks\\n",
                       (long long)n_entries, (long long)nc, (long long)run, (long long)c->walk_bases);
    tg.lap("[gpu thread]   classes");

    const int64_t n_words = (run + 31) / 32;
    PHICHK(phi_dev_ensure(c, c->d_wwords, (size_t)(n_words + 2) * 8));
    PHICHK(phi_dev_ensure(c, c->d_wbad, (size_t)(n_words + 6) * 4));
    auto pack = [&](uint8_t *ascii) {
        phi_launch_pack_classes(c->stream, c->d_seq.as<uint8_t>(), c->d_seq_off.as<int64_t>(), c->d_walk_vtx.as<int32_t>(), c->d_vlen.as<int32_t>(),
                                c->d_cls_rep.as<phi_ent_t>(), c->d_cls_left.as<uint8_t>(), c->d_cls_base.as<int64_t>(), nc,
                                c->d_wwords.as<uint64_t>(), n_words, c->d_wbad.as<uint32_t>(), ascii, (unsigned long long *)scalar(c, S_NBAD));
    };
    pack(nullptr);
    const uint8_t *cls_ascii = nullptr;
    {
        uint64_t n_bad = 0;
        HIPCHK(hipMemcpyAsync(&n_bad, scalar(c, S_NBAD), 8, hipMemcpyDeviceToHost, c->stream));
        HIPCHK(hipStreamSynchronize(c->stream));
        if (n_bad || c->k > PHI_MAX_K_PACKED) {
            PHICHK(phi_dev_ensure(c, c->d_wascii, (size_t)run + 64));
            HIPCHK(hipMemsetAsync(scalar(c, S_NBAD), 0, 8, c->stream));
            pack(c->d_wascii.as<uint8_t>());
            cls_ascii = c->d_wascii.as<uint8_t>();
        }
    }
    const size_t n_sw = (size_t)(run / 64 + 2);
    PHICHK(phi_dev_ensure(c, c->d_wstarts, n_sw * 8));
    HIPCHK(hipMemsetAsync(c->d_wstarts.p, 0, n_sw * 8, c->stream));
    phi_launch_mark_starts(c->stream, c->d_cls_base.as<int64_t>(), nc, c->d_wstarts.as<unsigned long long>());
    int64_t n_raw = 0;
    DevBuf raw_hash;
    PhiDevGuard guard1{{&raw_hash}};
    PHICHK(sketch_records(c, c->d_wwords.as<uint64_t>(), c->d_wstarts.as<unsigned long long>(), run, c->k, c->w, cls_ascii, raw_hash,
                          c->d_rec_pos, &n_raw));
    if (n_raw >= (int64_t)1 << 31) return phi_fail(c, PHI_ERR_UNSUPPORTED, "more than 2^31 minimisers in the distinct walk contexts");
    tg.lap("[gpu thread]   class-space pack + sketch");

    const int64_t nr0 = std::max<int64_t>(n_raw, 1);
    DevBuf r_cls, r_rel, r_e0, r_e1;
    PhiDevGuard guard4{{&r_cls, &r_rel, &r_e0, &r_e1}};
    PHICHK(phi_dev_ensure(c, r_cls, (size_t)nr0 * 4));
    PHICHK(phi_dev_ensure(c, r_rel, (size_t)nr0 * 4));
    PHICHK(phi_dev_ensure(c, r_e0, (size_t)nr0 * 4));
    PHICHK(phi_dev_ensure(c, r_e1, (size_t)nr0 * 4));
    PHICHK(phi_dev_ensure(c, c->d_flags, (size_t)std::max<int64_t>(nr0, n_entries)));
    phi_launch_class_rec(c->stream, c->d_rec_pos.as<int64_t>(), n_raw, c->d_cls_base.as<int64_t>(), nc, c->d_cls_rep.as<phi_ent_t>(),
                         c->d_cls_left.as<uint8_t>(), c->d_walk_vtx.as<int32_t>(), c->d_vlen.as<int32_t>(), c->k, c->d_flags.as<uint8_t>(),
                         r_cls.as<int32_t>(), r_rel.as<int32_t>(), r_e0.as<phi_ent_t>(), r_e1.as<phi_ent_t>());
    PHICHK(phi_compact(c, c->d_flags.as<uint8_t>(), n_raw, c->d_list2, &c->n_rec));
    const int64_t nr = std::max<int64_t>(c->n_rec, 1);
    PHICHK(phi_dev_ensure(c, c->d_rec_hash, (size_t)nr * 8));
    PHICHK(phi_dev_ensure(c, c->d_rec_cls, (size_t)nr * 4));
    PHICHK(phi_dev_ensure(c, c->d_rec_rel, (size_t)nr * 4));
    PHICHK(phi_dev_ensure(c, c->d_rec_e0, (size_t)nr * 4));
    PHICHK(phi_dev_ensure(c, c->d_rec_e1, (size_t)nr * 4));
    phi_launch_class_rec_gather(c->stream, c->d_list2.as<int32_t>(), c->n_rec, raw_hash.as<uint64_t>(), r_cls.as<int32_t>(), r_rel.as<int32_t>(),
                                r_e0.as<phi_ent_t>(), r_e1.as<phi_ent_t>(), c->d_rec_hash.as<uint64_t>(), c->d_rec_cls.as<int32_t>(),
                                c->d_rec_rel.as<int32_t>(), c->d_rec_e0.as<phi_ent_t>(), c->d_rec_e1.as<phi_ent_t>());
    phi_launch_class_rec_off(c->stream, c->d_rec_cls.as<int32_t>(), c->n_rec, nc, c->d_cls_rec_off.as<int32_t>());
    HIPCHK(hipEventRecord(ev1, c->stream));
    HIPCHK(hipStreamSynchronize(c->stream));
    float ms = 0.f;
    HIPCHK(hipEventElapsedTime(&ms, ev0, ev1));
    c->index_gpu_ms = ms;
    HIPCHK(hipGetLastError());
    return PHI_OK;
}

int set_graph_check_args(phi_ctx *c, int32_t n_vtx, const char *seq_concat, const int64_t *seq_off, const int64_t *adj_off,
                         const int32_t *adj, int32_t n_walks, const int64_t *walk_off, const int32_t *walk_vtx, const int32_t *topo_rank)
{
// ... 91 lines not shown
            PHICHK(phi_dev_ensure(c, c->d_g_off, (ne + 1) * 8));
            PHICHK(phi_dev_ensure(c, c->d_dmax, ne * 4));
            PHICHK(phi_dev_ensure(c, c->d_bstart, ne * 4));
            PHICHK(phi_dev_ensure(c, c->d_off_end, (ne + 3) * 4));
            PHICHK(phi_dev_ensure(c, c->d_off_start, (ne + 3) * 4));
            return PHI_OK;
        });
    }
}

static void start_uploads(SetGraph &S)
{
    S.uploads = std::async(std::launch::async, [&S]() -> int {
        phi_ctx *c = S.c;
        HIPCHK(hipSetDevice(c->device));
        PHICHK(upload(c, c->d_seq, S.seq_concat, (size_t)S.seq_off[S.n_vtx]));
        PHICHK(upload(c, c->d_seq_off, S.seq_off, (size_t)S.n_vtx + 1));
        if (!S.dev_walks) PHICHK(upload(c, c->d_walk_vtx, S.walk_vtx, (size_t)S.n_entries));
        PHICHK(upload(c, c->d_walk_off, S.walk_off, (size_t)S.n_walks + 1));
        PHICHK(upload(c, c->d_adj_off, S.adj_off, (size_t)S.n_vtx + 1));
        if (S.n_edges == 0) PHICHK(phi_dev_ensure(c, c->d_adj, 4));
        else PHICHK(upload(c, c->d_adj, S.adj, (size_t)S.n_edges));
        PHICHK(upload(c, c->d_topo_rank, S.topo_rank, (size_t)S.n_vtx));
        return PHI_OK;
    });
}

static int validate_topology(SetGraph &S)
{
    phi_ctx *c = S.c;
    PhiHostError verr;
    S.indeg.assign((size_t)S.n_vtx, 0);
    if (phi_topo_from_ranks(S.n_vtx, S.topo_rank, c->h_topo, verr) ||
        phi_check_edges(S.n_vtx, S.adj_off, S.adj, S.topo_rank, S.indeg.data(), verr))
        return phi_fail(c, verr.code, "%s", verr.msg.c_str());
    return PHI_OK;
}

static int start_host_walk_copy(SetGraph &S)
{
    phi_ctx *c = S.c;
    int64_t host_walks_max = (int64_t)1 << 26;
    if (const char *e = getenv("PHI_HOST_WALKS_MAX")) host_walks_max = atoll(e);
    S.keep_host_walks = S.n_entries <= host_walks_max;
    if (!c->h_walk_vtx.resize(S.keep_host_walks ? S.n_entries : 0)) return phi_fail(c, PHI_ERR_NOMEM, "host allocation failed");
    if (!S.keep_host_walks) return PHI_OK;
    S.wv_copy = std::async(std::launch::async, [c, dev_walks = S.dev_walks, n_entries = S.n_entries, walk_vtx = S.walk_vtx]() {
        int32_t *dst = c->h_walk_vtx.data();
        if (dev_walks) {
            (void)hipSetDevice(c->device);
            if (n_entries && hipMemcpyAsync(dst, c->d_walk_vtx.p, (size_t)n_entries * 4, hipMemcpyDeviceToHost, c->aux_stream) == hipSuccess)
                (void)hipStreamSynchronize(c->aux_stream);
            return;
        }
        const int nt = 4;
        std::vector<std::thread> th;
        for (int t = 0; t < nt; t++)
            th.emplace_back([=]() {
                const int64_t lo = n_entries * t / nt, hi = n_entries * (t + 1) / nt;
                memcpy(dst + lo, walk_vtx + lo, (size_t)(hi - lo) * 4);
            });
        for (auto &x : th) x.join();
    });
    return PHI_OK;
}

static int walk_entry_pass(SetGraph &S)
{
    phi_ctx *c = S.c;
    const int nw64 = c->dp_nw;
    PHICHK(phi_dev_ensure(c, c->d_e_out, (size_t)S.n_entries));
    PHICHK(phi_dev_ensure(c, c->d_cnt_edge, S.cnt_edge.size() * 4));
    PHICHK(phi_dev_ensure(c, c->d_walk_err, 16));
    HIPCHK(hipMemsetAsync(c->d_cnt_edge.p, 0, S.cnt_edge.size() * 4, c->stream));
    HIPCHK(hipMemsetAsync(c->d_walk_err.p, 0, 16, c->stream));
    if (S.want_masks) {
        PHICHK(phi_dev_ensure(c, c->d_st_mask, (size_t)S.n_vtx * nw64 * 8));
        HIPCHK(hipMemsetAsync(c->d_st_mask.p, 0, (size_t)S.n_vtx * nw64 * 8, c->stream));
    }
    phi_launch_walk_edges(c->stream, c->d_walk_vtx.as<int32_t>(), c->d_walk_off.as<int64_t>(), S.n_walks, S.n_entries, S.n_vtx,
                          c->d_adj_off.as<int64_t>(), c->d_adj.as<int32_t>(), c->d_seq_off.as<int64_t>(),
                          c->d_topo_rank.as<int32_t>(), c->d_e_out.as<uint8_t>(), c->d_cnt_edge.as<int32_t>(),
                          S.want_masks ? c->d_st_mask.as<unsigned long long>() : nullptr, nw64, c->d_walk_err.as<int32_t>());
    HIPCHK(hipMemcpyAsync(S.cnt_edge.data(), c->d_cnt_edge.p, S.cnt_edge.size() * 4, hipMemcpyDeviceToHost, c->stream));
    HIPCHK(hipMemcpyAsync(S.walk_err, c->d_walk_err.p, 16, hipMemcpyDeviceToHost, c->stream));
    HIPCHK(hipStreamSynchronize(c->stream));
    return PHI_OK;
}

static int build_minimizer_table(phi_ctx *c)
{
    const int64_t nr = std::max<int64_t>(c->n_rec, 1);
    PHICHK(phi_dev_ensure(c, c->d_rec_slot, (size_t)nr * 4));
    const uint64_t cap_full = pow2_at_least(std::max<uint64_t>(1024, 2 * (uint64_t)c->n_rec));
    const uint64_t UMULT = 8;
    PHICHK(phi_dev_ensure(c, c->d_flags, (size_t)nr));
    c->u_cap = cap_full;
    PHICHK(phi_dev_ensure(c, c->d_u_keys, c->u_cap * 8));
    PHICHK(phi_dev_ensure(c, c->d_u_rep, c->u_cap * 4));
    phi_launch_fill_u64(c->stream, c->d_u_keys.as<uint64_t>(), (int64_t)c->u_cap, PHI_EMPTY_KEY);
    phi_launch_fill_u32(c->stream, c->d_u_rep.as<uint32_t>(), (int64_t)c->u_cap, 0xFFFFFFFFu);
    phi_launch_table_build(c->stream, c->d_rec_hash.as<uint64_t>(), c->n_rec, c->d_u_keys.as<uint64_t>(),
                           c->d_u_rep.as<uint32_t>(), c->u_cap - 1, c->d_rec_slot.as<uint32_t>(),
                           (uint32_t *)scalar(c, S_ERR));
    phi_launch_rep_flags(c->stream, c->d_rec_slot.as<uint32_t>(), c->n_rec, c->d_u_rep.as<uint32_t>(),
                         c->d_flags.as<uint8_t>());
    PHICHK(phi_compact(c, c->d_flags.as<uint8_t>(), c->n_rec, c->d_u_replist, &c->n_unique));
    const uint64_t want = pow2_at_least(std::max<uint64_t>(1024, UMULT * (uint64_t)c->n_unique));
    if (c->u_cap > 2 * want || 2 * c->u_cap < want) {
        DevBuf keys2, uid2;
        PhiDevGuard guard{{&keys2, &uid2}};
        PHICHK(phi_dev_ensure(c, keys2, want * 8));
        PHICHK(phi_dev_ensure(c, uid2, want * 4));
        phi_launch_fill_u64(c->stream, keys2.as<uint64_t>(), (int64_t)want, PHI_EMPTY_KEY);
        phi_launch_table_compact(c->stream, c->d_u_replist.as<int32_t>(), c->n_unique, c->d_rec_hash.as<uint64_t>(), c->n_rec,
                                 keys2.as<uint64_t>(), uid2.as<uint32_t>(), want - 1, c->d_rec_slot.as<uint32_t>(),
                                 (uint32_t *)scalar(c, S_ERR));
        HIPCHK(hipStreamSynchronize(c->stream));
        phi_dev_free(c->d_u_keys); phi_dev_free(c->d_u_uid); phi_dev_free(c->d_u_rep);
        c->d_u_keys = keys2; c->d_u_uid = uid2;
        keys2 = DevBuf{}; uid2 = DevBuf{};
        c->u_cap = want;
    } else {
        PHICHK(phi_dev_ensure(c, c->d_u_uid, c->u_cap * 4));
        phi_launch_slot_uid(c->stream, c->d_u_replist.as<int32_t>(), c->n_unique, c->d_rec_slot.as<uint32_t>(),
                            c->d_u_uid.as<uint32_t>());
    }
    return PHI_OK;
}

static int gpu_thread(SetGraph &S)
{
    phi_ctx *c = S.c;
    struct PromiseGuard { std::promise<int> &p; bool done = false; ~PromiseGuard() { if (!done) p.set_value(PHI_ERR_DEVICE); } } pg{S.edges_promise};
    HIPCHK(hipSetDevice(c->device));
    PhiStageTimer tg("set_graph");
    PHICHK(S.uploads.get());
    {
        const int rc = walk_entry_pass(S);
        S.edges_promise.set_value(rc);
        pg.done = true;
        if (rc) return rc;
        if (tg.on) tg.lap("[gpu thread] uploads + walk-entry pass");
    }
    if (S.walk_err[0]) return PHI_OK;
    HIPCHK(hipMemsetAsync(c->d_scalars.p, 0, S_N * 8, c->stream));
    HIPCHK(hipMemsetAsync(c->d_stripes.p, 0, 2 * STRIPE_BYTES, c->stream));
    PHICHK(build_classes(c, S.n_vtx, S.n_walks, S.n_entries));
    c->h_kept = PhiAnchorSpan{}; c->h_dp = PhiAnchorSpan{}; c->anchors_host = false;
    if (tg.on) (void)hipStreamSynchronize(c->stream);
    tg.lap("[gpu thread] classes + class sketch");
    PHICHK(build_minimizer_table(c));
    PHICHK(build_read_table(c));
    PHICHK(phi_dev_ensure(c, c->d_list2, (size_t)(S.n_walks + 1) * 8));
    HIPCHK(hipMemsetAsync(c->d_list2.p, 0, (size_t)(S.n_walks + 1) * 8, c->stream));
    phi_launch_walk_rec_counts(c->stream, c->d_ent_cls.as<int32_t>(), c->d_cls_rec_off.as<int32_t>(), c->d_walk_off.as<int64_t>(),
                               S.n_walks, S.n_entries, c->d_list2.as<unsigned long long>());
    c->h_n_minimizers.assign(S.n_walks, 0);
    HIPCHK(hipMemcpyAsync(c->h_n_minimizers.data(), c->d_list2.p, (size_t)S.n_walks * 8, hipMemcpyDeviceToHost, c->stream));
    PHICHK(phi_dev_ensure(c, c->d_hit, (size_t)(c->n_unique / 8 + 1) * 8));
    HIPCHK(hipMemsetAsync(c->d_hit.p, 0, (size_t)(c->n_unique / 8 + 1) * 8, c->stream));
    PHICHK(phi_dev_ensure(c, c->alt.hit, (size_t)(c->n_unique / 8 + 1) * 8));
    HIPCHK(hipMemsetAsync(c->alt.hit.p, 0, (size_t)(c->n_unique / 8 + 1) * 8, c->stream));
    HIPCHK(hipMemsetAsync(c->alt.stripes.p, 0, 2 * STRIPE_BYTES, c->stream));
    HIPCHK(hipGetLastError());
    PHICHK(phi_sync_check(c));
    tg.lap("[gpu thread] walk sketch + table");
    return PHI_OK;
}

static void copy_graph_to_host(SetGraph &S)
{
    phi_ctx *c = S.c;
    std::thread t1([&]() { c->h_seq.assign(S.seq_concat, S.seq_concat + S.seq_off[S.n_vtx]); });
    std::thread t2([&]() { c->h_seq_off.assign(S.seq_off, S.seq_off + S.n_vtx + 1); });
    std::thread t3([&]() { c->h_adj_off.assign(S.adj_off, S.adj_off + S.n_vtx + 1); c->h_adj.assign(S.adj, S.adj + S.n_edges); });
    c->h_walk_off.assign(S.walk_off, S.walk_off + S.n_walks + 1);
    c->h_topo_rank.assign(S.topo_rank, S.topo_rank + S.n_vtx);
    t1.join(); t2.join(); t3.join();
}

static int report_walk_errors(SetGraph &S)
{
    phi_ctx *c = S.c;
    const int32_t *walk_err = S.walk_err;
    if (walk_err[0] == 4) return phi_fail(c, PHI_ERR_WALK, "walk %d holds vertex %d out of range", walk_err[1], walk_err[2]);
    if (walk_err[0] == 1) return phi_fail(c, PHI_ERR_UNSUPPORTED, "walk %d passes through empty segment %d", walk_err[1], walk_err[2]);
    if (walk_err[0] == 2) return phi_fail(c, PHI_ERR_WALK, "walk %d steps %d->%d without a graph edge", walk_err[1], walk_err[2], walk_err[3]);
    if (walk_err[0] == 3) return phi_fail(c, PHI_ERR_UNSUPPORTED, "vertex %d has more than 254 out-edges", walk_err[2]);
    return PHI_OK;
}

static int refuse_interior_ends(SetGraph &S)
{
    if (S.dev_walks) S.walk_ends = S.c->wtext.ends.data();
    else {
        S.ends_own.resize((size_t)S.n_walks * 2);
        for (int32_t h = 0; h < S.n_walks; h++) {
            S.ends_own[(size_t)h * 2] = S.walk_vtx[S.walk_off[h]];
            S.ends_own[(size_t)h * 2 + 1] = S.walk_vtx[S.walk_off[h + 1] - 1];
        }
        S.walk_ends = S.ends_own.data();
    }
    bool start_interior = false, end_interior = false;
    for (int32_t h = 0; h < S.n_walks; h++) {
        if (S.indeg[(size_t)S.walk_ends[(size_t)h * 2]] > 0) start_interior = true;
        const int32_t last = S.walk_ends[(size_t)h * 2 + 1];
        if (S.adj_off[last + 1] > S.adj_off[last]) end_interior = true;
    }
    if (start_interior && end_interior)
        return phi_fail(S.c, PHI_ERR_UNSUPPORTED, "walks both start and end at interior vertices: the reference model "
                        "admits flow leak/spawn artefacts there (ILP_index.cpp:1330) that are not emulated");
    return PHI_OK;
}

static int build_step_stream(SetGraph &S)
{
    phi_ctx *c = S.c;
    PhiStageTimer &tm = S.tm;
    const PhiDpGraph g{S.n_vtx, S.n_walks, S.adj_off, S.adj, S.topo_rank, c->h_topo.data(), S.cnt_edge.data(), S.walk_ends};
    PhiDpSteps &st = S.steps;
    PhiHostError err;
    if (phi_dp_steps_dense(g, st, err)) return phi_fail(c, err.code, "%s", err.msg.c_str());
    tm.lap("  dense step records");
    c->dp_events = S.n_walks <= PHI_DP_EVENT_MAX_WALKS && !getenv("PHI_DP_DENSE");
    c->n_k = 0; c->n_ev = 0;
    if (c->dp_events) {
        if (phi_dp_steps_compact(g, st, err)) return phi_fail(c, err.code, "%s", err.msg.c_str());
        c->n_k = st.n_k;
        if (tm.on) {
            int64_t n_tops = 0, n_entry = 0;
            for (int32_t k = 0; k < c->n_k; k++) { n_tops += (st.k_rec[(size_t)k * 8] & PHI_DP_NEED_TOPS) != 0; n_entry += (st.k_rec[(size_t)k * 8] & PHI_DP_NEED_ENTRY) != 0; }
            fprintf(stderr, "[phi timing] set_graph: %d compact steps: %lld with TOPS, %lld with ENTRY, %lld pairs\n", c->n_k, (long long)n_tops, (long long)n_entry, (long long)st.n_pairs);
        }
        tm.lap("  compact records");
        phi_dp_steps_cuts(st);
        c->h_cstep.swap(st.cstep); c->h_kstep.swap(st.kstep); c->h_k_cut_ok.swap(st.cut_ok);
        PHICHK(upload(c, c->d_k_rec, st.k_rec.data(), st.k_rec.size()));
        PHICHK(upload(c, c->d_k_in, st.k_in.data(), st.k_in.size()));
        PHICHK(upload(c, c->d_cvtx, st.cvtx.data(), st.cvtx.size()));
    }
    return PHI_OK;
}

static int late_uploads_and_events(SetGraph &S)
{
    phi_ctx *c = S.c;
    c->dp_dense_ready = S.want_masks;
    if (S.want_masks) {
        PHICHK(upload(c, c->d_st_rec, S.steps.st_rec.get(), (size_t)S.n_vtx * 8));
        PHICHK(upload(c, c->d_in_packed, S.steps.in_packed.data(), S.steps.in_packed.size()));
    }
    if (c->dp_events) {
        PHICHK(phi_dev_ensure(c, c->d_flags, (size_t)S.n_entries));
        phi_launch_event_flags(c->stream, c->d_walk_vtx.as<int32_t>(), S.n_entries, c->d_cvtx.as<int32_t>(), c->d_flags.as<uint8_t>());
        PHICHK(phi_compact(c, c->d_flags.as<uint8_t>(), S.n_entries, c->d_ev_e, &c->n_ev));
        if (c->n_ev >= (int64_t)1 << 31) return phi_fail(c, PHI_ERR_UNSUPPORTED, "more than 2^31 walk entries on vertices with recombination edges");
        PHICHK(phi_dev_ensure(c, c->d_ev_off, (size_t)(S.n_walks + 1) * 8));
        phi_launch_event_off(c->stream, c->d_ev_e.as<phi_ent_t>(), c->n_ev, c->d_walk_off.as<int64_t>(), S.n_walks,
                             c->d_ev_off.as<int64_t>());
    }
    HIPCHK(hipGetLastError());
    PHICHK(phi_sync_check(c));
    if (S.tm.on) fprintf(stderr, "[phi timing] set_graph: %d vertices, %d compact steps, %lld entries, %lld events\n", S.n_vtx, c->n_k, (long long)S.n_entries, (long long)c->n_ev);
    return PHI_OK;
}

static void reset_read_state(phi_ctx *c)
{
    c->reads_bases = 0; c->reads_count = 0; c->spectrum_override = -1;
    c->spset.new_graph(); c->rlog.new_generation(); c->rlog.async_batches = false;
    c->walks_on_device = false;
    c->rlog.nov_shift = phi_nov_shift(c->w);
    if (const char *e = getenv("PHI_NOV_SHIFT")) c->rlog.nov_shift = std::max(0, std::min(9, atoi(e)));
    c->alt.needs_clean = false;
}

int set_graph_impl(phi_ctx *c, int32_t n_vtx, const char *seq_concat, const int64_t *seq_off, const int64_t *adj_off,
                   const int32_t *adj, int32_t n_walks, const int64_t *walk_off, const int32_t *walk_vtx,
                   const int32_t *topo_rank)
{
    if (!c) return PHI_ERR_INVALID;
    PHICHK(set_graph_check_args(c, n_vtx, seq_concat, seq_off, adj_off, adj, n_walks, walk_off, walk_vtx, topo_rank));
    SetGraph S(c, n_vtx, seq_concat, seq_off, adj_off, adj, n_walks, walk_off, walk_vtx, topo_rank);
    PhiStageTimer &tm = S.tm;
    start_pinning(S);
    PHICHK(set_graph_check_offsets(c, n_vtx, seq_off, adj_off, n_walks, walk_off));
    S.n_edges = adj_off[n_vtx]; S.n_entries = walk_off[n_walks];
    start_dp_buffers(S);
    c->n_vtx = n_vtx; c->n_walks = n_walks; c->n_entries = S.n_entries;
    start_uploads(S);
    PHICHK(validate_topology(S));
    tm.lap("validate graph, copies");
    if (n_walks > PHI_DP_MAX_WALKS) return phi_fail(c, PHI_ERR_UNSUPPORTED, "more than %d walks", PHI_DP_MAX_WALKS);
    c->dp_nw = phi_dp_num_waves(n_walks);
    PHICHK(start_host_walk_copy(S));
    S.cnt_edge.assign((size_t)std::max<int64_t>(S.n_edges, 1), 0);
    S.want_masks = !(n_walks <= PHI_DP_EVENT_SAFE_WALKS && !getenv("PHI_DP_DENSE"));
    S.gpu = std::async(std::launch::async, [&S]() { return gpu_thread(S); });
    copy_graph_to_host(S);
    tm.lap("host copies");
    PHICHK(S.edges_future.get());
    PHICHK(report_walk_errors(S));
    tm.lap("walk entries: pass on the GPU");
    PHICHK(refuse_interior_ends(S));
    PHICHK(build_step_stream(S));
// ... 80 lines not shown
```

### phi_amd/csrc/sketch_dev.h

```cpp
#pragma once
#include <hip/hip_runtime.h>
#include <type_traits>
#include <hip/hip_ext.h>
#include "phi_dev.h"
#include "phi_kernels.h"
#ifndef PHI_ABL
#define PHI_ABL 0
#endif

#define TPB PHI_TPB
#define Q 8


static __device__ __forceinline__ void pack_ascii_word(int64_t wi, const uint8_t *__restrict__ bases, int64_t n,
                                                       uint64_t *__restrict__ words, int64_t n_words,
                                                       uint32_t *__restrict__ badbits,
                                                       unsigned long long *__restrict__ n_bad)
{
    if (wi >= n_words + 4) return;
    if (wi >= n_words) {
        if (wi < n_words + 2) words[wi] = 0;
        if (badbits) badbits[wi] = 0;
        return;
    }
    const int64_t b0 = wi * 32;
    uint64_t word = 0;
    uint32_t bad = 0;
    if (b0 + 32 <= n && ((uintptr_t)(bases + b0) & 15) == 0) {
        const uint4 *p = reinterpret_cast<const uint4 *>(bases + b0);
        uint4 v[2] = {p[0], p[1]};
        const uint32_t *u = reinterpret_cast<const uint32_t *>(v);
#pragma unroll
        for (int q = 0; q < 8; q++) {
#pragma unroll
            for (int j = 0; j < 4; j++) {
                const uint32_t c = (u[q] >> (8 * j)) & 0xFFu;
                bad |= (uint32_t)(!phi_is_acgt(c)) << (4 * q + j);
                word = (word << 2) | phi_code(c);
            }
        }
    } else {
        for (int j = 0; j < 32; j++) {
            uint32_t c = 'A';
            if (b0 + j < n) { c = bases[b0 + j]; bad |= (uint32_t)(!phi_is_acgt(c)) << j; }
            word = (word << 2) | phi_code(c);
        }
    }
    words[wi] = word;
    if (badbits) badbits[wi] = bad;
    if (bad) atomicAdd(n_bad, (unsigned long long)__popc(bad));
}

static __device__ __forceinline__ void start_bitmap_word(int64_t j, const int64_t *__restrict__ seq_off, int64_t n_seq,
                                                         unsigned long long *__restrict__ starts, int64_t n_sw, int64_t total = 0)
{
    if (j >= n_sw) return;
    const int64_t lo_b = j * 64, hi_b = lo_b + 64;
    int64_t lo = 0, hi = n_seq;
    if (total > 0 && n_seq > 64) {
        int64_t g = (int64_t)((double)lo_b / (double)total * (double)n_seq);
        g = g < 0 ? 0 : (g > n_seq - 1 ? n_seq - 1 : g);
        if (seq_off[g] >= lo_b) {
            hi = g;
            int64_t step = 1;
            while (hi - step >= 0) {
                if (seq_off[hi - step] < lo_b) { lo = hi - step + 1; break; }
                hi -= step;
                step <<= 1;
            }
        } else {
            lo = g + 1;
            int64_t step = 1;
            while (lo + step < n_seq) {
                if (seq_off[lo + step] >= lo_b) { hi = lo + step; break; }
                lo += step + 1;
                step <<= 1;
            }
        }
    }
    while (lo < hi) {
        const int64_t mid = (lo + hi) >> 1;
        if (seq_off[mid] < lo_b) lo = mid + 1; else hi = mid;
    }
    unsigned long long word = 0;
    for (int64_t r = lo; r < n_seq; r++) {
        const int64_t p = seq_off[r];
        if (p >= hi_b) break;
        if (seq_off[r + 1] > p) word |= 1ull << (p & 63);
    }
    starts[j] = word;
}


__device__ __forceinline__ void wave_sync()
{
    __builtin_amdgcn_fence(__ATOMIC_ACQ_REL, "wavefront");
    __builtin_amdgcn_wave_barrier();
}

__device__ __forceinline__ int next_start_lds(const unsigned long long *s_bits, int from, int limit)
{
    if (from >= limit) return INT_MAX;
    int wi = from >> 6;
    const int wl = (limit - 1) >> 6;
    unsigned long long word = s_bits[wi] & (~0ull << (from & 63));
    for (;;) {
        if (word) {
            const int p = (wi << 6) + (__ffsll((long long)word) - 1);
            return p < limit ? p : INT_MAX;
        }
        if (++wi > wl) return INT_MAX;
        word = s_bits[wi];
    }
}

__device__ __forceinline__ uint64_t lds_extract64(const uint64_t *s_words, int lb)
{
    const int wi = lb >> 5, s = (lb & 31) * 2;
    return (s_words[wi] << s) | ((s_words[wi + 1] >> 1) >> (63 - s));
}

struct MinEnt { uint64_t v; int i; };
__device__ __forceinline__ MinEnt take_right(MinEnt a, MinEnt b) { return (b.v <= a.v) ? b : a; }

struct ProbeArgs { const uint64_t *u_rt; uint64_t u_bmask; uint8_t *hit; uint32_t *err; };
__device__ __forceinline__ void rt_bucket(const uint64_t *rt, uint64_t b, ulonglong2 &s0, uint3 &s1)
{
    const uint64_t *p = rt + 4 * b;
    s0 = *reinterpret_cast<const ulonglong2 *>(p);
    s1 = *reinterpret_cast<const uint3 *>(p + 2);
    asm volatile("" : "+v"(s0.x), "+v"(s0.y), "+v"(s1.x), "+v"(s1.y), "+v"(s1.z));
}
__device__ __forceinline__ bool probe_table(const ProbeArgs &A, uint64_t h)
{
    if (h == PHI_EMPTY_KEY) { atomicOr(A.err, PHI_KERR_SENTINEL); return false; }
    uint64_t b = h & A.u_bmask;
    ulonglong2 s0;
    uint3 s1;
    rt_bucket(A.u_rt, b, s0, s1);
    const uint64_t k1 = ((uint64_t)s1.y << 32) | s1.x;
    if (s0.x == h) { A.hit[(uint32_t)s0.y] = 1; return false; }
    if (k1 == h) { A.hit[s1.z] = 1; return false; }
    if ((s0.y >> 32) & PHI_RT_OVERFLOWED) {
        for (int probes = 1; probes <= PHI_MAX_PROBE; probes++) {
            b = (b + 1) & A.u_bmask;
            rt_bucket(A.u_rt, b, s0, s1);
            const uint64_t n1 = ((uint64_t)s1.y << 32) | s1.x;
            if (s0.x == h) { A.hit[(uint32_t)s0.y] = 1; return false; }
            if (n1 == h) { A.hit[s1.z] = 1; return false; }
            if (n1 == PHI_EMPTY_KEY) break;
        }
    }
    return true;
}

__device__ __forceinline__ bool probe_table(const PhiSketchArgs &A, uint64_t h)
{
    const ProbeArgs P{A.u_rt, A.u_bmask, A.hit, A.err};
    return probe_table(P, h);
}

struct OverflowArgs { uint64_t *list; unsigned long long *count; int64_t cap; uint32_t *err; };
__device__ __forceinline__ int overflow_novel(const OverflowArgs &O, bool ov, uint64_t h, int lane)
{
    const unsigned long long ob = __ballot(ov);
    if (!ob) return 0;
    const int first = __ffsll((long long)ob) - 1, n = __popcll(ob);
    unsigned long long base = 0;
    if (lane == first) base = atomicAdd(O.count, (unsigned long long)n);
    base = __shfl(base, first, 64);
    if (ov) {
        const unsigned long long idx = base + (unsigned long long)__popcll(ob & ((1ull << lane) - 1));
        if ((int64_t)idx < O.cap) O.list[idx] = h;
        else atomicOr(O.err, PHI_KERR_TABLE_FULL);
    }
    return n;
}
typedef const __attribute__((address_space(4))) PhiSketchArgs *KArgs;
__device__ __forceinline__ KArgs kargs_now()
{
    KArgs p = (KArgs)__builtin_amdgcn_kernarg_segment_ptr();
    asm volatile("" : "+s"(p));
    return p;
}


struct KRef { int64_t pos; int rc; };

__device__ __forceinline__ uint32_t up_byte(uint32_t c) { return (c >= 'a' && c <= 'z') ? c - 32 : c; }
__device__ __forceinline__ uint32_t comp_byte(uint32_t c)
{
    return c == 'A' ? 'T' : c == 'T' ? 'A' : c == 'C' ? 'G' : c == 'G' ? 'C' : c;
}
__device__ __forceinline__ uint32_t kbyte(const uint8_t *__restrict__ s, KRef r, int x, int k)
{
    return r.rc ? comp_byte(up_byte(s[r.pos + k - 1 - x])) : up_byte(s[r.pos + x]);
}
__device__ __forceinline__ int kcmp(const uint8_t *__restrict__ s, KRef a, KRef b, int k)
{
    for (int x = 0; x < k; x++) {
        const uint32_t ca = kbyte(s, a, x, k), cb = kbyte(s, b, x, k);
        if (ca != cb) return ca < cb ? -1 : 1;
    }
    return 0;
}
__device__ __forceinline__ KRef canon_bytes(const uint8_t *__restrict__ s, int64_t i, int k)
{
    const KRef f{i, 0}, r{i, 1};
    return kcmp(s, r, f, k) < 0 ? r : f;
}
__device__ KRef window_best_bytes(const uint8_t *__restrict__ s, int64_t a, int k, int w)
{
    KRef best = canon_bytes(s, a, k);
    for (int j = 1; j < w; j++) {
        const KRef c = canon_bytes(s, a + j, k);
        if (kcmp(s, c, best, k) <= 0) best = c;
    }
    return best;
}
template <bool LONGK>
__device__ uint64_t khash_bytes(const uint8_t *__restrict__ s, KRef r, int k)
{
    if (LONGK && k > PHI_MAX_K_PACKED) {
        uint64_t e[8] = {0, 0, 0, 0, 0, 0, 0, 0};
        for (int g = 0; g < 8; g++) {
            uint64_t v = 0;
            for (int x = 8 * g; x < 8 * g + 8 && x < k; x++) v |= (uint64_t)kbyte(s, r, x, k) << (8 * (x & 7));
            e[g] = v;
        }
        return phi_murmur_lanes8(e, k);
    }
    uint64_t e0 = 0, e1 = 0, e2 = 0, e3 = 0;
    for (int x = 0; x < k; x++) {
        const uint64_t b = (uint64_t)kbyte(s, r, x, k) << (8 * (x & 7));
        if (x < 8) e0 |= b; else if (x < 16) e1 |= b; else if (x < 24) e2 |= b; else e3 |= b;
    }
    return phi_murmur_lanes(e0, e1, e2, e3, k);
}

__device__ __forceinline__ bool range_has_bit(const unsigned long long *s_bits, int lo, int hi)
{
    return next_start_lds(s_bits, lo, hi + 1) != INT_MAX;
}

template <int MODE, bool LONGK = false>
__device__ __forceinline__ void slow_windows(const PhiSketchArgs &A, int64_t c0, int64_t chunk, int lane, int k, int w,
                                          const unsigned long long *s_bits, const unsigned long long *s_bad,
                                          bool allslow, int64_t out_base, int &n_emit, int &n_nov)
{
    const int64_t N = A.n_bases;
    const int span = w + k - 1;
    for (int r = 0; r < PHI_WCH / 64; r++) {
        const int la = 1 + r * 64 + lane;
        const int64_t a = c0 - 1 + la;
        const int lp = la + 63;
        bool todo = (a + span <= N) && !range_has_bit(s_bits, lp + 1, lp + span - 1);
        if (todo && !allslow) todo = range_has_bit(s_bad, lp - 1, lp + span - 1);
        bool emit = false;
        uint64_t h = 0;
        int64_t pos = 0;
        if (todo) {
            const bool first = (s_bits[lp >> 6] >> (lp & 63)) & 1ull;
            const KRef best = window_best_bytes(A.ascii, a, k, w);
            h = khash_bytes<LONGK>(A.ascii, best, k);
            pos = best.pos;
            if (first) emit = h != PHI_EMPTY_KEY;
            else {
                const KRef prev = window_best_bytes(A.ascii, a - 1, k, w);
                emit = !(prev.pos == best.pos && prev.rc == best.rc) && khash_bytes<LONGK>(A.ascii, prev, k) != h;
            }
        }
        const unsigned long long bal = __ballot(emit);
        bool novel = false;
        if (emit) {
            const int rank = n_emit + __popcll(bal & ((1ull << lane) - 1));
            if (MODE == PHI_MODE_WRITE) {
                A.out_hash[out_base + rank] = h;
                A.out_pos[out_base + rank] = pos;
            } else if (MODE == PHI_MODE_PROBE) {
                novel = probe_table(A, h);
            }
        }
        if (MODE == PHI_MODE_PROBE) {
            const OverflowArgs O{A.ov_list, A.ov_count, A.ov_cap, A.err};
            n_nov += overflow_novel(O, novel, h, lane);
        }
        n_emit += __popcll(bal);
    }
// ... 261 lines not shown
```

### phi_amd/csrc/sketch_win_fixed.hip

```cpp
#include "sketch_dev.h"

__device__ __forceinline__ uint32_t revcomp16(uint32_t x)
{
    x = __builtin_bitreverse32(x);
    return ~(((x >> 1) & 0x55555555u) | ((x << 1) & 0xAAAAAAAAu));
}

template <int S>
__device__ __forceinline__ uint64_t bits62(uint32_t u0, uint32_t u1, uint32_t u2)
{
    static_assert(S >= 0 && S <= 34, "inside the 96 bits");
    uint32_t lo, hi;
    if constexpr (S >= 32) {
        lo = __builtin_amdgcn_alignbit(u0, u1, S - 32);
        hi = (u0 >> (S - 32)) & 0x3FFFFFFFu;
    } else {
        lo = __builtin_amdgcn_alignbit(u1, u2, S);
        hi = __builtin_amdgcn_alignbit(u0, u1, S) & 0x3FFFFFFFu;
    }
    return ((uint64_t)hi << 32) | lo;
}

template <int KT, int WT, int LT>
__global__ void __launch_bounds__(TPB, 7) phi_sketch_winfix_kernel(PhiSketchArgs A)
{
    constexpr int MODE = PHI_MODE_PROBE;
    constexpr bool NEED_POS = false, WIDE = true, FMIN = true;
    constexpr int k = KT, w = WT, L = LT, span = w + k - 1, V = L - span + 1;
    constexpr int G = (V + Q - 1) / Q, s = G + (w + Q - 1) / Q, R = 64 / G;
    constexpr int NKM = L - k + 1, P = NKM / G;
    static_assert(k == 31 && w > Q, "31-mers: values below 2^62, two 62-bit extracts of 48 bases");
    static_assert(V == Q * G && NKM == P * G && P == 10, "every window and k-mer of a lane exists; the store offsets below");
    static_assert(R * L <= 928 && R * G <= 64, "the staging of phase 0");
    extern __shared__ uint64_t s_dyn[];

    const int lane = threadIdx.x & 63, wid = threadIdx.x >> 6;
    const int64_t chunk = (int64_t)blockIdx.x * (TPB / 64) + wid;
    const int64_t rd0 = chunk * R;
    const int64_t c0 = (rd0 * L) & ~(int64_t)31;
    const int64_t N = A.n_bases;
    const uint4 bv = load_bases16<1>(A.ascii, N, c0, lane);
    if (A.ipc_mb && chunk == 0 && lane == 0)
        __hip_atomic_store(A.ipc_mb + PHI_MB_SCORED, A.ipc_scored, __ATOMIC_RELEASE, __HIP_MEMORY_SCOPE_AGENT);
    if (rd0 >= A.n_reads) {
        if (A.q_clean) clean_finish(A, chunk, (int64_t)gridDim.x * (TPB / 64), lane);
        return;
    }
    const int nr = A.n_reads - rd0 < R ? (int)(A.n_reads - rd0) : R;
    const int rl = (int)((unsigned)lane / (unsigned)G), j = lane - rl * G;
    const bool live = rl < nr;

    using MetaT = uint16_t;
    constexpr uint32_t ITEM_FIRST = 1u << 15;
    constexpr uint32_t ITEM_NOEMIT = 1u << 14;
    uint64_t *s_mp = s_dyn + (size_t)wid * phi_win_region_u64(R, s, w, k);
    uint32_t *s_code = (uint32_t *)s_mp;
    unsigned long long *s_bad = (unsigned long long *)s_mp;
    MetaT *s_meta = (MetaT *)(s_mp + 9 * (64 + 1));
    uint64_t *s_q = s_mp + (live ? 9 * (rl * s + j) : 0);

    bool chunk_bad;
    {
        const uint32_t x[4] = {bv.x, bv.y, bv.z, bv.w};
        uint32_t code = 0, bad = 0;
#pragma unroll
        for (int q = 0; q < 4; q++) {
            const uint32_t t = ((x[q] >> 1) ^ (x[q] >> 2)) & 0x03030303u;
            const uint32_t c8 = (t * 0x40100401u) >> 24;
            code = (code << 8) | c8;
            if (__builtin_amdgcn_perm(0x54474341u, 0x54474341u, t) != (x[q] & 0xDFDFDFDFu)) {
#pragma unroll
                for (int b = 0; b < 4; b++) bad |= (uint32_t)(!phi_is_acgt((x[q] >> (8 * b)) & 0xFFu)) << (4 * q + b);
            }
        }
        s_code[lane] = code;
        chunk_bad = __ballot(lane < 62 && bad != 0) != 0ull;
    }
    wave_sync();

    {
        const int lb = (int)((rd0 * L) & 31) + rl * L + P * j + 32;
        const int d0 = (lb - 1) >> 4, rsh = 30 - 2 * ((lb - 1) & 15);
        const uint32_t d[4] = {s_code[d0], s_code[d0 + 1], s_code[d0 + 2], s_code[d0 + 3]};
        wave_sync();
        const uint32_t u0 = __builtin_amdgcn_alignbit(d[0], d[1], rsh);
        const uint32_t u1 = __builtin_amdgcn_alignbit(d[1], d[2], rsh);
        const uint32_t u2 = __builtin_amdgcn_alignbit(d[2], d[3], rsh);
        const uint32_t z0 = revcomp16(u2), z1 = revcomp16(u1), z2 = revcomp16(u0);
        uint64_t km[P];
#define KM(i) km[i] = min_u62(bits62<34 - 2 * (i)>(u0, u1, u2), bits62<2 * (i)>(z0, z1, z2))
        KM(0); KM(1); KM(2); KM(3); KM(4); KM(5); KM(6); KM(7); KM(8); KM(9);
#undef KM
        if (live) {
            const int u = 8 * s * rl + 1 + P * j, m = j & 3;
            uint64_t *b0 = s_mp + u + (u >> 3);
            uint64_t *b1 = b0 + (m == 3), *b2 = b0 + (m >= 2), *b3 = b0 + (m >= 1);
            b0[0] = km[0];
            b1[1] = km[1]; b1[2] = km[2];
            b2[3] = km[3]; b2[4] = km[4];
            b3[5] = km[5]; b3[6] = km[6];
            b0[8] = km[7]; b0[9] = km[8];
            b1[10] = km[9];
        }
    }
    wave_sync();

#include "sketch_minima.inc"

    if (chunk_bad) {
        wave_sync();
        stage_bad_bits(A.ascii, N, c0, lane, s_bad);
        wave_sync();
    }
    uint32_t cflag = 0, fflag = 0, pflag = 0;
    if (live) {
        constexpr uint32_t in_read = (2u << Q) - 2u;
        const uint32_t first = j == 0 ? 2u : 0u;
        uint32_t changed = 0;
#pragma unroll
        for (int i = 1; i <= Q; i++) changed |= (uint32_t)(wv[i] != wv[i - 1]) << i;
        uint32_t dall = 0, reseed = 0;
        if (chunk_bad) {
            const int lp0 = (int)((rd0 * L) & 31) + rl * L + Q * j - 1 + 64;
            for (int i = 0; i <= Q; i++) dall |= (uint32_t)range_has_bit(s_bad, lp0 + i - 1, lp0 + i + span - 1) << i;
            reseed = ~dall & (dall << 1);
        }
        cflag = in_read & ~dall & (first | changed | reseed);
        fflag = cflag & first;
        pflag = cflag & reseed & ~first;
    }
    int ncand, coff;
    {
        const int cnt = __popc(cflag) + __popc(pflag);
        const int v = wave_scan_inclusive(cnt);
        ncand = __builtin_amdgcn_readlane(v, 63);
        coff = v - cnt;
    }
    wave_sync();
    {
        uint64_t *s_w = s_mp + 9 * lane;
#define SW(x) s_w[(x) + ((x) >> 3)]
        if (lane == 0) SW(0) = wv[0];
#pragma unroll
        for (int i = 1; i <= Q; i++) SW(i) = wv[i];
#undef SW
        int c = coff + 1;
        if (!chunk_bad) {
            for (uint32_t f = cflag; f; f &= f - 1) {
                const uint32_t i = (uint32_t)__ffs((int)f) - 1;
                s_meta[c++] = (MetaT)((uint32_t)(lane * Q) + i + (((fflag >> i) & 1u) ? ITEM_FIRST : 0u));
            }
        } else {
#pragma unroll
            for (int i = 1; i <= Q; i++) {
                if ((cflag >> i) & 1u) {
                    if ((pflag >> i) & 1u) s_meta[c++] = (MetaT)((uint32_t)(lane * Q + i - 1) | ITEM_NOEMIT);
                    s_meta[c++] = (MetaT)((uint32_t)(lane * Q + i) | (((fflag >> i) & 1u) ? ITEM_FIRST : 0u));
                }
            }
        }
        if (coff == 0 && cflag) s_meta[0] = (MetaT)((uint32_t)(lane * Q + __ffs((int)cflag) - 2) | ITEM_NOEMIT);
    }
    wave_sync();
#undef SQ

    int n_emit = 0, n_log = 0, n_nov_slow = 0;
    const int64_t out_base = 0;
#include "sketch_rounds.inc"

    if (chunk_bad) {
        unsigned long long *s_bad_s = (unsigned long long *)(s_dyn + (size_t)__builtin_amdgcn_readfirstlane(wid) * phi_win_region_u64(R, s, w, k));
        wave_sync();
        stage_bad_bits(A.ascii, N, c0, lane, s_bad_s);
        wave_sync();
        int n_emit_slow = 0;
        slow_windows_reads(A, rd0, nr, L, V, c0, lane, k, w, s_bad_s, n_emit_slow, n_nov_slow);
        n_emit += n_emit_slow;
    }
    {
        const KArgs PA = kargs_now();
        if (PA->q_clean) clean_finish(*PA, chunk, (int64_t)gridDim.x * (TPB / 64), lane);
        if (lane == 0) {
            const int cap = 1 << PA->nov_shift;
            PA->nov_cnt[PA->log_base + chunk] = (uint16_t)(n_log < cap ? n_log : cap);
            const int n_nov_wave = n_log + n_nov_slow;
            const int stripe = (int)(chunk & (PHI_STRIPES - 1)) * 8;
            if (n_nov_wave && PA->n_logged) atomicAdd(PA->n_logged + stripe, (unsigned long long)n_nov_wave);
            if (n_emit && PA->n_emitted) atomicAdd(PA->n_emitted + stripe, (unsigned long long)n_emit);
        }
    }
}

bool phi_launch_sketch_win_fixed(hipStream_t st, unsigned nb, size_t lds, const PhiSketchArgs &A, hipEvent_t t0, hipEvent_t t1)
{
    if (!(A.k == 31 && A.w == 25 && A.uniform_len == 150 && A.win_reads == 5)) return false;
    if (const char *e = getenv("PHI_SKETCH_WIN_FIXED"))
        if (!atoi(e)) return false;
    hipExtLaunchKernelGGL((phi_sketch_winfix_kernel<31, 25, 150>), dim3(nb), dim3(TPB), lds, st, t0, t1, 0, A);
    return true;
}
```

### phi_amd/csrc/table.hip

```cpp
#include <hip/hip_runtime.h>
#include "phi_dev.h"
#include "phi_kernels.h"
#include "phi_wave.h"

__global__ void phi_fill_u64_kernel(uint64_t *p, int64_t n, uint64_t v)
{
    for (int64_t i = (int64_t)blockIdx.x * blockDim.x + threadIdx.x; i < n; i += (int64_t)gridDim.x * blockDim.x)
        p[i] = v;
}
__global__ void phi_fill_u32_kernel(uint32_t *p, int64_t n, uint32_t v)
{
    for (int64_t i = (int64_t)blockIdx.x * blockDim.x + threadIdx.x; i < n; i += (int64_t)gridDim.x * blockDim.x)
        p[i] = v;
}

static inline unsigned grid_for(int64_t n, int tpb)
{
    int64_t nb = (n + tpb - 1) / tpb;
    if (nb > 256 * 16) nb = 256 * 16;
    if (nb < 1) nb = 1;
    return (unsigned)nb;
}

__global__ void __launch_bounds__(256) phi_read_table_clear_kernel(ulonglong2 *__restrict__ rt, int64_t n_slots)
// ... 71 lines not shown
            if (++probes > PHI_MAX_PROBE) { atomicOr(err, PHI_KERR_TABLE_FULL); break; }
        }
        if (__builtin_nontemporal_load(&u_rep[slot]) > (uint32_t)i) atomicMin(&u_rep[slot], (uint32_t)i);
        rec_slot[i] = (uint32_t)slot;
    }
}

void phi_launch_table_build(hipStream_t st, const uint64_t *rec_hash, int64_t n_rec, uint64_t *u_keys,
                            uint32_t *u_rep, uint64_t u_mask, uint32_t *rec_slot, uint32_t *err)
{
    if (n_rec > 0)
        hipLaunchKernelGGL(phi_table_build_kernel, dim3(grid_for(n_rec, 256)), dim3(256), 0, st, rec_hash, n_rec,
                           u_keys, u_rep, u_mask, rec_slot, err);
}

__global__ void __launch_bounds__(256) phi_rep_flags_kernel(const uint32_t *__restrict__ rec_slot, int64_t n_rec,
                                                            const uint32_t *__restrict__ u_rep,
                                                            uint8_t *__restrict__ flags)
{
    for (int64_t i = (int64_t)blockIdx.x * blockDim.x + threadIdx.x; i < n_rec; i += (int64_t)gridDim.x * blockDim.x)
        flags[i] = u_rep[rec_slot[i]] == (uint32_t)i;
}
__global__ void __launch_bounds__(256) phi_slot_uid_kernel(const int32_t *__restrict__ rep_list, int64_t n_unique,
                                                           const uint32_t *__restrict__ rec_slot,
                                                           uint32_t *__restrict__ u_uid)
{
    for (int64_t j = (int64_t)blockIdx.x * blockDim.x + threadIdx.x; j < n_unique; j += (int64_t)gridDim.x * blockDim.x)
        u_uid[rec_slot[rep_list[j]]] = (uint32_t)j;
}
void phi_launch_rep_flags(hipStream_t st, const uint32_t *rec_slot, int64_t n_rec, const uint32_t *u_rep,
                          uint8_t *flags)
{
    if (n_rec > 0)
        hipLaunchKernelGGL(phi_rep_flags_kernel, dim3(grid_for(n_rec, 256)), dim3(256), 0, st, rec_slot, n_rec, u_rep,
                           flags);
}
void phi_launch_slot_uid(hipStream_t st, const int32_t *rep_list, int64_t n_unique, const uint32_t *rec_slot,
                         uint32_t *u_uid)
{
    if (n_unique > 0)
        hipLaunchKernelGGL(phi_slot_uid_kernel, dim3(grid_for(n_unique, 256)), dim3(256), 0, st, rep_list, n_unique,
                           rec_slot, u_uid);
}

__global__ void __launch_bounds__(256) phi_table_compact_insert_kernel(const int32_t *__restrict__ rep_list, int64_t n_unique,
                                                                       const uint64_t *__restrict__ rec_hash,
                                                                       uint64_t *__restrict__ keys, uint32_t *__restrict__ uid,
                                                                       uint64_t mask, uint32_t *__restrict__ err)
{
    for (int64_t i = (int64_t)blockIdx.x * blockDim.x + threadIdx.x; i < n_unique; i += (int64_t)gridDim.x * blockDim.x) {
        const uint64_t h = rec_hash[rep_list[i]];
        uint64_t slot = h & mask;
        int probes = 0;
        for (;;) {
            const unsigned long long prev = atomicCAS((unsigned long long *)&keys[slot], PHI_EMPTY_KEY, h);
            if (prev == PHI_EMPTY_KEY) break;
            slot = (slot + 1) & mask;
            if (++probes > PHI_MAX_PROBE) { atomicOr(err, PHI_KERR_TABLE_FULL); break; }
        }
        uid[slot] = (uint32_t)i;
    }
}

__global__ void __launch_bounds__(256) phi_table_lookup_kernel(const uint64_t *__restrict__ rec_hash, int64_t n_rec,
                                                               const uint64_t *__restrict__ keys, uint64_t mask,
                                                               uint32_t *__restrict__ rec_slot, uint32_t *__restrict__ err)
{
    for (int64_t i = (int64_t)blockIdx.x * blockDim.x + threadIdx.x; i < n_rec; i += (int64_t)gridDim.x * blockDim.x) {
        const uint64_t h = rec_hash[i];
        uint64_t slot = h & mask;
        int probes = 0;
        while (keys[slot] != h) {
            slot = (slot + 1) & mask;
            if (++probes > PHI_MAX_PROBE) { atomicOr(err, PHI_KERR_TABLE_FULL); break; }
        }
        rec_slot[i] = (uint32_t)slot;
    }
}

void phi_launch_table_compact(hipStream_t st, const int32_t *rep_list, int64_t n_unique, const uint64_t *rec_hash, int64_t n_rec,
                              uint64_t *keys, uint32_t *uid, uint64_t mask, uint32_t *rec_slot, uint32_t *err)
{
    if (n_unique > 0)
        hipLaunchKernelGGL(phi_table_compact_insert_kernel, dim3(grid_for(n_unique, 256)), dim3(256), 0, st, rep_list, n_unique,
                           rec_hash, keys, uid, mask, err);
    if (n_rec > 0)
        hipLaunchKernelGGL(phi_table_lookup_kernel, dim3(grid_for(n_rec, 256)), dim3(256), 0, st, rec_hash, n_rec, keys, mask,
                           rec_slot, err);
}

__global__ void __launch_bounds__(256) phi_share_hist_kernel(const uint64_t *__restrict__ keys, int64_t cap,
                                                             const int32_t *__restrict__ n_walks_of,
                                                             unsigned long long *__restrict__ hist)
{
    for (int64_t s = (int64_t)blockIdx.x * blockDim.x + threadIdx.x; s < cap; s += (int64_t)gridDim.x * blockDim.x)
        if (keys[s] != PHI_EMPTY_KEY) atomicAdd(&hist[n_walks_of[s]], 1ull);
}

void phi_launch_share_hist(hipStream_t st, const uint64_t *keys, int64_t cap, const int32_t *n_walks_of, unsigned long long *hist)
{
    if (cap > 0)
        hipLaunchKernelGGL(phi_share_hist_kernel, dim3(grid_for(cap, 256)), dim3(256), 0, st, keys, cap, n_walks_of, hist);
}

__global__ void __launch_bounds__(256) phi_spectrum_insert_kernel(const uint64_t *__restrict__ hashes, int64_t n,
                                                                  uint64_t *__restrict__ sp_keys, uint64_t sp_mask,
                                                                  unsigned long long *__restrict__ sp_count,
                                                                  const uint64_t *__restrict__ u_keys, uint64_t u_mask,
                                                                  const uint32_t *__restrict__ u_uid, uint8_t *__restrict__ hit,
                                                                  uint32_t *__restrict__ err)
{
    int n_new = 0;
    for (int64_t i = (int64_t)blockIdx.x * blockDim.x + threadIdx.x; i < n; i += (int64_t)gridDim.x * blockDim.x) {
        const uint64_t h = hashes[i];
        if (h == PHI_EMPTY_KEY) continue;
        if (u_keys) {
            bool found = false;
            uint64_t su = h & u_mask;
            for (int probes = 0; probes <= PHI_MAX_PROBE; probes++) {
                const uint64_t key = u_keys[su];
                if (key == h) { hit[u_uid[su]] = 1; found = true; break; }
                if (key == PHI_EMPTY_KEY) break;
                su = (su + 1) & u_mask;
            }
            if (found) continue;
        }
        uint64_t slot = h & sp_mask;
        int probes = 0;
        for (;;) {
            const unsigned long long prev = atomicCAS((unsigned long long *)&sp_keys[slot], PHI_EMPTY_KEY, h);
            if (prev == PHI_EMPTY_KEY) { n_new++; break; }
            if (prev == h) break;
            slot = (slot + 1) & sp_mask;
            if (++probes > PHI_MAX_PROBE) { atomicOr(err, PHI_KERR_TABLE_FULL); break; }
        }
    }
    n_new = phi_wave_sum(n_new);
    if ((threadIdx.x & 63) == 0 && n_new)
        atomicAdd(sp_count + (size_t)((blockIdx.x * 4 + (threadIdx.x >> 6)) & (PHI_STRIPES - 1)) * 8, (unsigned long long)n_new);
}

void phi_launch_spectrum_insert(hipStream_t st, const uint64_t *hashes, int64_t n, uint64_t *sp_keys,
                                uint64_t sp_mask, unsigned long long *sp_count, const uint64_t *u_keys, uint64_t u_mask,
                                const uint32_t *u_uid, uint8_t *hit, uint32_t *err)
{
    if (n > 0)
        hipLaunchKernelGGL(phi_spectrum_insert_kernel, dim3(grid_for(n, 256)), dim3(256), 0, st, hashes, n, sp_keys,
                           sp_mask, sp_count, u_keys, u_mask, u_uid, hit, err);
}

__global__ void __launch_bounds__(256) phi_spectrum_flush_kernel(const uint64_t *__restrict__ nov_log, const uint16_t *__restrict__ nov_cnt,
                                                                 int64_t c_lo, int64_t n_ent, int32_t shift,
                                                                 uint64_t *__restrict__ sp_keys, uint64_t sp_mask,
                                                                 unsigned long long *__restrict__ sp_count, uint32_t *__restrict__ err)
{
    int n_new = 0;
    for (int64_t t = (int64_t)blockIdx.x * blockDim.x + threadIdx.x; t < n_ent; t += (int64_t)gridDim.x * blockDim.x) {
        const int64_t c = c_lo + (t >> shift);
        const int i = (int)(t & ((1 << shift) - 1));
        if (i >= (int)nov_cnt[c]) continue;
        const uint64_t h = __builtin_nontemporal_load(&nov_log[(c << shift) + i]);
        uint64_t slot = h & sp_mask;
        int probes = 0;
        for (;;) {
            const unsigned long long prev = atomicCAS((unsigned long long *)&sp_keys[slot], PHI_EMPTY_KEY, h);
            if (prev == PHI_EMPTY_KEY) { n_new++; break; }
            if (prev == h) break;
            slot = (slot + 1) & sp_mask;
            if (++probes > PHI_MAX_PROBE) { atomicOr(err, PHI_KERR_TABLE_FULL); break; }
        }
    }
    n_new = phi_wave_sum(n_new);
    if ((threadIdx.x & 63) == 0 && n_new)
        atomicAdd(sp_count + (size_t)((blockIdx.x * 4 + (threadIdx.x >> 6)) & (PHI_STRIPES - 1)) * 8, (unsigned long long)n_new);
}

void phi_launch_spectrum_flush(hipStream_t st, const uint64_t *nov_log, const uint16_t *nov_cnt, int64_t c_lo, int64_t c_hi, int32_t shift,
                               uint64_t *sp_keys, uint64_t sp_mask, unsigned long long *sp_count, uint32_t *err)
{
    const int64_t n_ent = (c_hi - c_lo) << shift;
    if (n_ent > 0)
        hipLaunchKernelGGL(phi_spectrum_flush_kernel, dim3(grid_for(n_ent, 256)), dim3(256), 0, st, nov_log, nov_cnt, c_lo, n_ent, shift,
                           sp_keys, sp_mask, sp_count, err);
}

__global__ void __launch_bounds__(256) phi_count_flags_kernel(const uint8_t *__restrict__ flags, int64_t n,
                                                              unsigned long long *__restrict__ n_out)
{
    int cnt = 0;
    for (int64_t i = (int64_t)blockIdx.x * blockDim.x + threadIdx.x; i < n; i += (int64_t)gridDim.x * blockDim.x)
        cnt += flags[i] != 0;
    cnt = phi_wave_sum(cnt);
    if ((threadIdx.x & 63) == 0 && cnt) atomicAdd(n_out, (unsigned long long)cnt);
}

void phi_launch_count_flags(hipStream_t st, const uint8_t *flags, int64_t n, unsigned long long *n_out)
{
    if (n > 0) hipLaunchKernelGGL(phi_count_flags_kernel, dim3(grid_for(n, 256)), dim3(256), 0, st, flags, n, n_out);
}

__global__ void __launch_bounds__(256) phi_spectrum_export_kernel(const uint64_t *__restrict__ sp_keys, int64_t cap,
                                                                  uint64_t *__restrict__ out,
                                                                  unsigned long long *__restrict__ n_out)
{
    for (int64_t i0 = (int64_t)blockIdx.x * blockDim.x; i0 < cap; i0 += (int64_t)gridDim.x * blockDim.x) {
        const int64_t i = i0 + threadIdx.x;
        const uint64_t key = i < cap ? sp_keys[i] : PHI_EMPTY_KEY;
        const bool occ = key != PHI_EMPTY_KEY;
        const unsigned long long bal = __ballot(occ);
        const int lane = threadIdx.x & 63;
        unsigned long long base = 0;
        if (lane == 0 && bal) base = atomicAdd(n_out, (unsigned long long)__popcll(bal));
        base = __shfl(base, 0, 64);
        if (occ) out[base + __popcll(bal & ((1ull << lane) - 1))] = key;
    }
}

void phi_launch_spectrum_export(hipStream_t st, const uint64_t *sp_keys, int64_t cap, uint64_t *out,
                                unsigned long long *n_out)
{
    if (cap > 0)
        hipLaunchKernelGGL(phi_spectrum_export_kernel, dim3(grid_for(cap, 256)), dim3(256), 0, st, sp_keys, cap, out,
                           n_out);
}

__global__ void phi_warm_table_kernel() {}
void phi_warm_table(hipStream_t st) { hipLaunchKernelGGL(phi_warm_table_kernel, dim3(1), dim3(64), 0, st); }
```

Before: 451.5.

## Key read sketch lookups by mixed canonical k-mer instead of MurmurHash

Builds a second read table at graph setup, keyed by an invertible mix of each walk minimiser's canonical 2-bit k-mer. Clean read chunks can then look up k-mers directly and skip per-window MurmurHash3 in the hot sketch rounds. Novel entries are logged as raw k-mers and hashed later in the flush kernel, which also checks that no two distinct k-mers share a hash. The path is on by default when the chunk count fits a CU-derived bound. The cost is extra table memory, more setup work, and a new error when a hash collision is found.

```diff
diff --git a/phi_amd/build.py b/phi_amd/build.py
--- a/phi_amd/build.py
+++ b/phi_amd/build.py
@@ -8,7 +8,7 @@
 ARCH = "gfx950"
 
 HIP_SOURCES = ["sketch.hip", "sketch_pooled.hip", "sketch_win_fixed.hip", "table.hip", "anchors.hip", "contexts.hip", "dp.hip", "dp_events.hip", "phi_abi.hip", "dev_mem.hip", "read_batches.hip", "text_stream.hip", "text_park.hip", "set_graph.hip", "phi_solve.hip", "solve_dev.hip", "phi_comm.hip", "phi_ipc.hip", "reads_text.hip", "walk_text.hip", "edit.hip", "edit_path.hip", "inflate.hip", "gfa_text.hip", "chop.hip", "vcf.hip", "ladder.hip", "panel.hip", "panel_score.hip", "scan.hip", "bam.hip", "calls.hip"]
-HIP_HEADERS = ["phi_dev.h", "phi_kernels.h", "phi_ctx.h", "phi_dp_flags.h", "phi_host_par.h", "phi_wave.h", "dp_steps.h", "solve_host.h", "reads_host.h", "bam_header.h", "sketch_dev.h", "sketch_phases.inc", "sketch_minima.inc", "sketch_rounds.inc", "edit_band.inc", os.path.join("host", "panel_choose.h"), os.path.join("..", "..", "include", "phi_amd.h")]
+HIP_HEADERS = ["phi_dev.h", "phi_kernels.h", "phi_ctx.h", "phi_dp_flags.h", "phi_host_par.h", "phi_wave.h", "dp_steps.h", "solve_host.h", "reads_host.h", "bam_header.h", "sketch_dev.h", "sketch_phases.inc", "sketch_minima.inc", "sketch_rounds.inc", "sketch_rounds_kmer.inc", "edit_band.inc", os.path.join("host", "panel_choose.h"), os.path.join("..", "..", "include", "phi_amd.h")]
 
 
 def _run(cmd, cwd=None):
diff --git a/phi_amd/csrc/host/kmer_keys_selftest.cpp b/phi_amd/csrc/host/kmer_keys_selftest.cpp
--- /dev/null
+++ b/phi_amd/csrc/host/kmer_keys_selftest.cpp
@@ -0,0 +1,75 @@
+#include <stdint.h>
+#include <stdio.h>
+#include "../phi_dev.h"
+
+static int n_failed = 0;
+static void line(const char *name, bool ok, const char *what)
+{
+    printf("%s %s %s\n", name, ok ? "ok" : "FAILED", what);
+    if (!ok) n_failed++;
+}
+
+static uint64_t rng_state = 0x243F6A8885A308D3ull;
+static uint64_t rnd()
+{
+    uint64_t z = (rng_state += 0x9E3779B97F4A7C15ull);
+    z = (z ^ (z >> 30)) * 0xBF58476D1CE4E5B9ull;
+    z = (z ^ (z >> 27)) * 0x94D049BB133111EBull;
+    return z ^ (z >> 31);
+}
+
+int main()
+{
+    char buf[256];
+    {
+        long bad = 0;
+        for (int i = 0; i < 1000000; i++) {
+            const uint64_t x = rnd();
+            bad += phi_kmer_unmix(phi_kmer_mix(x)) != x;
+            bad += phi_kmer_mix(phi_kmer_unmix(x)) != x;
+        }
+        snprintf(buf, sizeof buf, "random=1000000 bad=%ld", bad);
+        line("inverse_random", bad == 0, buf);
+    }
+    {
+        const uint64_t edge[3] = {0ull, (1ull << 62) - 1, ~0ull};
+        bool ok = true;
+        for (uint64_t x : edge) ok = ok && phi_kmer_unmix(phi_kmer_mix(x)) == x;
+        line("inverse_edges", ok, "0, 2^62 - 1, ~0");
+    }
+    {
+        const uint64_t pre = phi_kmer_unmix(PHI_EMPTY_KEY);
+        snprintf(buf, sizeof buf, "preimage=0x%016llx", (unsigned long long)pre);
+        line("sentinel_preimage", pre >= (1ull << 62) && phi_kmer_mix(pre) == PHI_EMPTY_KEY, buf);
+        line("multiplier_inverse", (uint64_t)(PHI_KMER_MIX_MUL * PHI_KMER_MIX_INV) == 1ull, "mul * inv == 1 mod 2^64");
+    }
+    {
+        int taken_hi = 0, taken_lo = 0;
+        static uint8_t hi[1 << 16], lo[1 << 16];
+        for (uint64_t i = 0; i < (1u << 16); i++) {
+            uint8_t &a = hi[phi_kmer_mix((i << 46) | 0x2AAAAAAAAAAull) & 0xFFFF], &b = lo[phi_kmer_mix((0x1555ull << 46) | i) & 0xFFFF];
+            taken_hi += !a; a = 1;
+            taken_lo += !b; b = 1;
+        }
+        snprintf(buf, sizeof buf, "taken_hi=%d taken_lo=%d of 65536", taken_hi, taken_lo);
+        line("low_bits_mixed", taken_hi > 36000 && taken_lo > 36000, buf);
+    }
+    const uint64_t H = 0x0123456789ABCDEFull, V = 0x1B1B1B1B1B1B1Bull, V2 = 0x2C2C2C2C2C2C2Cull;
+    line("rule_plain_first", phi_kmer_flush_rule(H, V, false, 0, 0, false) == 0, "first entry of a chunk, not a walk hash: inserted");
+    line("rule_plain_prev_differs", phi_kmer_flush_rule(H, V, true, H + 1, V2, false) == 0, "another k-mer with another hash before it: inserted");
+    line("rule_same_kmer_twice", phi_kmer_flush_rule(H, V, true, H, V, false) == 0, "the same k-mer before it (the next read's first window): inserted");
+    line("rule_novel_novel", phi_kmer_flush_rule(H, V, true, H, V2, false) == PHI_KERR_HASH_COLLISION, "equal hash, different k-mer before it: collision");
+    line("rule_novel_novel_no_prev", phi_kmer_flush_rule(H, V, false, H, V2, false) == 0, "the same pair without a predecessor (entry 0): hp, vp ignored");
+    line("rule_novel_walk", phi_kmer_flush_rule(H, V, false, 0, 0, true) == PHI_KERR_HASH_COLLISION, "the hash of a novel k-mer is a walk minimiser's: collision");
+    line("rule_both", phi_kmer_flush_rule(H, V, true, H, V2, true) == PHI_KERR_HASH_COLLISION, "both at once: one bit");
+    line("rule_sentinel", phi_kmer_flush_rule(PHI_EMPTY_KEY, V, false, 0, 0, false) == PHI_KERR_SENTINEL, "h == PHI_EMPTY_KEY: sentinel");
+    line("rule_sentinel_first", phi_kmer_flush_rule(PHI_EMPTY_KEY, V, true, PHI_EMPTY_KEY, V2, true) == PHI_KERR_SENTINEL, "the sentinel goes before everything else");
+    line("error_bits", PHI_KERR_HASH_COLLISION == 128u && PHI_KERR_SENTINEL == 1u, "128, 1");
+    {
+        uint64_t v = 0;
+        for (int i = 0; i < 31; i++) v = (v << 2) | (uint64_t)(i & 3);
+        const uint64_t e0 = 0x5447434154474341ull, e3 = 0x0047434154474341ull;
+        line("hash_of_value", phi_kmer_hash(v, 31) == phi_murmur_lanes(e0, e0, e0, e3, 31), "phi_kmer_hash(v) == murmur of the spelled bytes");
+    }
+    return n_failed ? 1 : 0;
+}
diff --git a/phi_amd/csrc/phi_abi.hip b/phi_amd/csrc/phi_abi.hip
--- a/phi_amd/csrc/phi_abi.hip
+++ b/phi_amd/csrc/phi_abi.hip
@@ -131,7 +131,7 @@
     DevBuf *all[] = {&c->d_anchors, &c->d_cov_all, &c->d_cov_w, &c->d_slots, &c->d_slots2, &c->d_segs, &c->d_ctr, &c->d_vmax, &c->d_lane_walk, &c->d_walk_lane, &c->d_coff, &c->d_blk_ncls, &c->d_rownew, &c->d_blk_bad, &c->d_seg_lo, &c->d_seg_row, &c->d_seg_S, &c->wtext.d_text, &c->panel.d_full, &c->scout.d_scores, &c->d_sel_off, &c->d_sel_tri, &c->d_blk_lo, &c->d_blk_ev, &c->d_blk_S, &c->d_row_out, &c->d_rowend, &c->d_blk_keys, &c->d_blk_carry, &c->d_cov, &c->d_cov2, &c->d_stepdiff, &c->alt.hit, &c->hit_extra[0], &c->hit_extra[1], &c->alt.stripes, &c->spset.d_sp_cnt, &c->rlog.d_novlog, &c->rlog.d_novcnt, &c->rlog.d_ovlist, &c->d_vlen, &c->d_ent_cls, &c->d_cls_rep, &c->d_cls_left, &c->d_cls_mult, &c->d_cls_base, &c->d_cls_rec_off, &c->d_rec_cls, &c->d_rec_rel, &c->d_u_replist, &c->d_adj_off, &c->d_adj, &c->d_topo_rank, &c->d_cnt_edge, &c->d_walk_err, &c->d_sa_cnt, &c->d_sa_cur, &c->d_sa_off, &c->d_sa_idx, &c->d_seq, &c->d_seq_off, &c->d_walk_vtx, &c->d_walk_off, &c->d_topo, &c->d_in_off,
                      &c->d_in_src, &c->d_e_out, &c->d_st_rec, &c->d_st_mask, &c->d_in_packed, &c->d_word, &c->d_wwords, &c->d_wbad,
                      &c->d_wascii, &c->d_wstarts, &c->d_rec_hash, &c->d_rec_pos, &c->d_rec_slot,
-                     &c->d_rec_e0, &c->d_rec_e1, &c->d_u_keys, &c->d_u_rep, &c->d_u_uid, &c->d_rt, &c->d_in_s, &c->d_last_walk, &c->d_rowdiag, &c->d_wpre, &c->d_hit, &c->spset.d_sp_keys, &c->d_rbases,
+                     &c->d_rec_e0, &c->d_rec_e1, &c->d_u_keys, &c->d_u_rep, &c->d_u_uid, &c->d_rt, &c->d_kt, &c->d_in_s, &c->d_last_walk, &c->d_rowdiag, &c->d_wpre, &c->d_hit, &c->spset.d_sp_keys, &c->d_rbases,
                      &c->d_roff, &c->rlog.d_roff_made, &c->d_peer_send, &c->spset.d_export, &c->d_scalars, &c->d_stripes, &c->d_blk_cnt,
                      &c->d_blk_off, &c->d_flags, &c->d_flags2, &c->d_list, &c->d_list2, &c->d_list3, &c->d_walk_last, &c->d_m_rec, &c->d_m_group,
                      &c->d_g_keys, &c->d_g_rep, &c->d_g_cnt, &c->d_slot_maxcnt, &c->d_slot_multi, &c->d_a_e1,
diff --git a/phi_amd/csrc/phi_ctx.h b/phi_amd/csrc/phi_ctx.h
--- a/phi_amd/csrc/phi_ctx.h
+++ b/phi_amd/csrc/phi_ctx.h
@@ -120,6 +120,9 @@
     DevBuf d_u_keys, d_u_rep, d_u_uid, d_u_replist;
     DevBuf d_rt;
     uint64_t rt_buckets = 0, rt_mask = 0;
+    DevBuf d_kt;
+    uint64_t kt_buckets = 0, kt_mask = 0;
+    int64_t kt_max_chunks = 0;
     void *h_stage[2] = {nullptr, nullptr};
     hipEvent_t stage_ev[2] = {nullptr, nullptr};
     DevBuf d_wpre;
diff --git a/phi_amd/csrc/phi_dev.h b/phi_amd/csrc/phi_dev.h
--- a/phi_amd/csrc/phi_dev.h
+++ b/phi_amd/csrc/phi_dev.h
@@ -193,3 +193,29 @@
     }
     return phi_murmur_lanes(e[0], e[1], e[2], e[3], k);
 }
+
+#define PHI_KMER_MIX_MUL 0x9E3779B97F4A7C15ull
+#define PHI_KMER_MIX_INV 0xF1DE83E19937733Dull
+PHI_HD uint64_t phi_kmer_mix(uint64_t v)
+{
+    v ^= v >> 31;
+    v = phi_mul64(v, PHI_KMER_MIX_MUL);
+    return v ^ (v >> 32);
+}
+PHI_HD uint64_t phi_kmer_unmix(uint64_t y)
+{
+    y ^= y >> 32;
+    y = y * PHI_KMER_MIX_INV;
+    return y ^ (y >> 31) ^ (y >> 62);
+}
+
+#define PHI_KERR_SENTINEL 1u
+#define PHI_KERR_HASH_COLLISION 128u
+PHI_HD uint32_t phi_kmer_flush_rule(uint64_t h, uint64_t v, bool have_prev, uint64_t hp, uint64_t vp, bool in_walks)
+{
+    if (h == PHI_EMPTY_KEY) return PHI_KERR_SENTINEL;
+    uint32_t e = 0;
+    if (in_walks) e |= PHI_KERR_HASH_COLLISION;
+    if (have_prev && hp == h && vp != v) e |= PHI_KERR_HASH_COLLISION;
+    return e;
+}
diff --git a/phi_amd/csrc/phi_kernels.h b/phi_amd/csrc/phi_kernels.h
--- a/phi_amd/csrc/phi_kernels.h
+++ b/phi_amd/csrc/phi_kernels.h
@@ -38,6 +38,7 @@
 #define PHI_KERR_CSR_ID 32u
 #define PHI_KERR_DP_QUEUE 16u
 #define PHI_KERR_DP_CLASSES 64u
+#define PHI_KERR_HASH_COLLISION 128u
 
 struct PhiSketchArgs {
     const uint64_t *words;
@@ -69,7 +70,9 @@
     unsigned long long *ov_zero;
     unsigned long long *ipc_mb; unsigned long long ipc_scored, ipc_need;
     uint64_t *q_hit_words; int64_t q_n_hit_words; uint64_t *q_stripes; int64_t q_n_stripe_words;
-};
+    const uint64_t *k_rt; uint64_t k_bmask;
+};
+#define PHI_NOV_KMERS 0x8000u
 
 void phi_launch_pack_ascii(hipStream_t st, const uint8_t *bases, int64_t n, uint64_t *words, int64_t n_words,
                            uint32_t *badbits, unsigned long long *n_bad);
@@ -100,7 +103,12 @@
                                 uint64_t sp_mask, unsigned long long *sp_count, const uint64_t *u_keys, uint64_t u_mask,
                                 const uint32_t *u_uid, uint8_t *hit, uint32_t *err);
 void phi_launch_spectrum_flush(hipStream_t st, const uint64_t *nov_log, const uint16_t *nov_cnt, int64_t c_lo, int64_t c_hi, int32_t shift,
-                               uint64_t *sp_keys, uint64_t sp_mask, unsigned long long *sp_count, uint32_t *err);
+                               uint64_t *sp_keys, uint64_t sp_mask, unsigned long long *sp_count, int32_t k, const uint64_t *u_keys,
+                               uint64_t u_mask, uint32_t *err);
+void phi_launch_kmer_keys(hipStream_t st, const int32_t *rec_cls, const int32_t *rec_rel, const uint64_t *rec_hash, const uint32_t *rec_slot,
+                          int64_t n_rec, const int64_t *cls_base, const uint8_t *cls_left, const uint64_t *words, const uint32_t *badbits,
+                          int32_t k, uint64_t *kkeys, unsigned long long *ctr);
+void phi_launch_rt_overflowed(hipStream_t st, const uint64_t *rt, int64_t n_buckets, unsigned long long *n_out);
 void phi_launch_count_flags(hipStream_t st, const uint8_t *flags, int64_t n, unsigned long long *n_out);
 void phi_launch_spectrum_export(hipStream_t st, const uint64_t *sp_keys, int64_t cap, uint64_t *out,
                                 unsigned long long *n_out);
diff --git a/phi_amd/csrc/read_batches.hip b/phi_amd/csrc/read_batches.hip
--- a/phi_amd/csrc/read_batches.hip
+++ b/phi_amd/csrc/read_batches.hip
@@ -107,7 +107,8 @@
         PHICHK(sp_reserve(c, in_set, more));
         if (L.log_chunks > L.log_done)
             phi_launch_spectrum_flush(c->stream, L.d_novlog.as<uint64_t>(), L.d_novcnt.as<uint16_t>(), L.log_done, L.log_chunks, L.nov_shift,
-                                      S.d_sp_keys.as<uint64_t>(), S.sp_cap - 1, S.d_sp_cnt.as<unsigned long long>(), (uint32_t *)scalar(c, S_ERR));
+                                      S.d_sp_keys.as<uint64_t>(), S.sp_cap - 1, S.d_sp_cnt.as<unsigned long long>(), c->k, c->d_u_keys.as<uint64_t>(),
+                                      c->u_cap - 1, (uint32_t *)scalar(c, S_ERR));
         if ((int64_t)ov_now > L.ov_done)
             phi_launch_spectrum_insert(c->stream, L.d_ovlist.as<uint64_t>() + L.ov_done, (int64_t)ov_now - L.ov_done, S.d_sp_keys.as<uint64_t>(),
                                        S.sp_cap - 1, S.d_sp_cnt.as<unsigned long long>(), nullptr, 0, nullptr, nullptr, (uint32_t *)scalar(c, S_ERR));
@@ -143,6 +144,7 @@
     const uint32_t err = (uint32_t)s[S_ERR];
     if (err & PHI_KERR_TABLE_FULL) return phi_fail(c, PHI_ERR_OVERFLOW, "open-addressed table overflow (probe bound %d), or the overflow list of novel read hashes ran full under a batch handed over with phi_add_reads_device", PHI_MAX_PROBE);
     if (err & PHI_KERR_SENTINEL) return phi_fail(c, PHI_ERR_UNSUPPORTED, "a minimiser hashes to UINT64_MAX (table sentinel)");
+    if (err & PHI_KERR_HASH_COLLISION) return phi_fail(c, PHI_ERR_UNSUPPORTED, "two different k-mers of the reads and walks share a MurmurHash3 value: the k-mer route cannot reproduce the reference's result for this read set (set PHI_SKETCH_KMER_KEYS=0 and run again)");
     return PHI_OK;
 }
 
@@ -217,6 +219,11 @@
     A.u_rt = c->d_rt.as<uint64_t>(); A.u_bmask = c->rt_mask;
     A.hit = c->d_hit.as<uint8_t>();
     A.err = (uint32_t *)scalar(c, S_ERR);
+    if (c->kt_mask) {
+        const char *e = getenv("PHI_SKETCH_KMER_KEYS");
+        const int mode = e ? atoi(e) : 1;
+        if (mode >= 2 || (mode == 1 && n_log_chunks <= c->kt_max_chunks)) { A.k_rt = c->d_kt.as<uint64_t>(); A.k_bmask = c->kt_mask; }
+    }
     A.nov_log = L.d_novlog.as<uint64_t>(); A.nov_cnt = L.d_novcnt.as<uint16_t>(); A.log_base = L.log_chunks; A.nov_shift = L.nov_shift;
     A.ov_list = L.d_ovlist.as<uint64_t>(); A.ov_cap = L.ov_cap;
     A.ov_count = (unsigned long long *)scalar(c, S_OVCNT + (int)(c->spset.sp_gen % 3));
diff --git a/phi_amd/csrc/set_graph.hip b/phi_amd/csrc/set_graph.hip
--- a/phi_amd/csrc/set_graph.hip
+++ b/phi_amd/csrc/set_graph.hip
@@ -27,6 +27,59 @@
         nb *= 2;
     }
     c->rt_buckets = nb; c->rt_mask = nb - 1;
+    return PHI_OK;
+}
+
+static int build_kmer_table(phi_ctx *c)
+{
+    c->kt_buckets = 0; c->kt_mask = 0;
+    if (c->k > 31 || c->n_rec <= 0 || c->n_unique <= 0) return PHI_OK;
+    PhiStageTimer tg("set_graph");
+    DevBuf kkeys, ctr;
+    PhiDevGuard guard{{&kkeys, &ctr}};
+    PHICHK(phi_dev_ensure(c, kkeys, c->u_cap * 8));
+    PHICHK(phi_dev_ensure(c, ctr, 5 * 8));
+    phi_launch_fill_u64(c->stream, kkeys.as<uint64_t>(), (int64_t)c->u_cap, PHI_EMPTY_KEY);
+    HIPCHK(hipMemsetAsync(ctr.p, 0, 5 * 8, c->stream));
+    phi_launch_kmer_keys(c->stream, c->d_rec_cls.as<int32_t>(), c->d_rec_rel.as<int32_t>(), c->d_rec_hash.as<uint64_t>(), c->d_rec_slot.as<uint32_t>(),
+                         c->n_rec, c->d_cls_base.as<int64_t>(), c->d_cls_left.as<uint8_t>(), c->d_wwords.as<uint64_t>(), c->d_wbad.as<uint32_t>(),
+                         c->k, kkeys.as<uint64_t>(), ctr.as<unsigned long long>());
+    uint64_t n[5] = {0, 0, 0, 0, 0};
+    HIPCHK(phi_copy_sync(c, n, ctr.p, 3 * 8, hipMemcpyDeviceToHost));
+    if (n[1]) return phi_fail(c, PHI_ERR_DEVICE, "k-mer table: %llu class records whose k-mer in class space does not hash to the record's hash (internal error)", (unsigned long long)n[1]);
+    if (n[2]) {
+        if (tg.on) fprintf(stderr, "[phi timing] set_graph: %llu walk minimisers share a hash with another k-mer: no k-mer table for this graph\n", (unsigned long long)n[2]);
+        return PHI_OK;
+    }
+    uint64_t nb = c->rt_buckets;
+    uint32_t err0 = 0;
+    HIPCHK(phi_copy_sync(c, &err0, scalar(c, S_ERR), 4, hipMemcpyDeviceToHost));
+    if (err0 & PHI_KERR_TABLE_FULL) return PHI_OK;
+    for (int attempt = 0;; attempt++) {
+        PHICHK(phi_dev_ensure(c, c->d_kt, nb * 32));
+        phi_launch_read_table(c->stream, kkeys.as<uint64_t>(), c->d_u_uid.as<uint32_t>(), (int64_t)c->u_cap, c->d_kt.as<uint64_t>(), (int64_t)nb,
+                              (uint32_t *)scalar(c, S_ERR));
+        uint32_t err = 0;
+        HIPCHK(phi_copy_sync(c, &err, scalar(c, S_ERR), 4, hipMemcpyDeviceToHost));
+        if (!(err & PHI_KERR_TABLE_FULL)) break;
+        if (attempt >= 40) return phi_fail(c, PHI_ERR_OVERFLOW, "k-mer table overflow at %llu buckets (internal error)", (unsigned long long)nb);
+        err &= ~PHI_KERR_TABLE_FULL;
+        HIPCHK(phi_copy_sync(c, scalar(c, S_ERR), &err, 4, hipMemcpyHostToDevice));
+        nb *= 2;
+    }
+    c->kt_buckets = nb; c->kt_mask = nb - 1;
+    int n_cu = 0;
+    HIPCHK(hipDeviceGetAttribute(&n_cu, hipDeviceAttributeMultiprocessorCount, c->device));
+    c->kt_max_chunks = (int64_t)n_cu * 4 * 7;
+    if (tg.on) {
+        phi_launch_rt_overflowed(c->stream, c->d_rt.as<uint64_t>(), (int64_t)c->rt_buckets, ctr.as<unsigned long long>() + 3);
+        phi_launch_rt_overflowed(c->stream, c->d_kt.as<uint64_t>(), (int64_t)nb, ctr.as<unsigned long long>() + 4);
+        HIPCHK(phi_copy_sync(c, n + 3, ctr.as<uint64_t>() + 3, 2 * 8, hipMemcpyDeviceToHost));
+        fprintf(stderr, "[phi timing] set_graph: k-mer table of %llu buckets (%.1f MB) beside the read table's %llu; %llu class records with a base outside ACGT skipped; "
+                        "OVERFLOWED buckets: read table %.2e, k-mer table %.2e\n", (unsigned long long)nb, (double)nb * 32 / 1e6, (unsigned long long)c->rt_buckets,
+                (unsigned long long)n[0], (double)n[3] / (double)c->rt_buckets, (double)n[4] / (double)nb);
+        tg.lap("[gpu thread]   k-mer table");
+    }
     return PHI_OK;
 }
 
@@ -424,6 +477,7 @@
     tg.lap("[gpu thread] classes + class sketch");
     PHICHK(build_minimizer_table(c));
     PHICHK(build_read_table(c));
+    PHICHK(build_kmer_table(c));
     PHICHK(phi_dev_ensure(c, c->d_list2, (size_t)(S.n_walks + 1) * 8));
     HIPCHK(hipMemsetAsync(c->d_list2.p, 0, (size_t)(S.n_walks + 1) * 8, c->stream));
     phi_launch_walk_rec_counts(c->stream, c->d_ent_cls.as<int32_t>(), c->d_cls_rec_off.as<int32_t>(), c->d_walk_off.as<int64_t>(),
diff --git a/phi_amd/csrc/sketch_dev.h b/phi_amd/csrc/sketch_dev.h
--- a/phi_amd/csrc/sketch_dev.h
+++ b/phi_amd/csrc/sketch_dev.h
@@ -131,9 +131,10 @@
     s1 = *reinterpret_cast<const uint3 *>(p + 2);
     asm volatile("" : "+v"(s0.x), "+v"(s0.y), "+v"(s1.x), "+v"(s1.y), "+v"(s1.z));
 }
+template <bool SENT = true>
 __device__ __forceinline__ bool probe_table(const ProbeArgs &A, uint64_t h)
 {
-    if (h == PHI_EMPTY_KEY) { atomicOr(A.err, PHI_KERR_SENTINEL); return false; }
+    if (SENT && h == PHI_EMPTY_KEY) { atomicOr(A.err, PHI_KERR_SENTINEL); return false; }
     uint64_t b = h & A.u_bmask;
     ulonglong2 s0;
     uint3 s1;
diff --git a/phi_amd/csrc/sketch_rounds_kmer.inc b/phi_amd/csrc/sketch_rounds_kmer.inc
--- /dev/null
+++ b/phi_amd/csrc/sketch_rounds_kmer.inc
@@ -0,0 +1,24 @@
+    if (ncand > 0) {
+        const ProbeArgs KP{A.k_rt, A.k_bmask, A.hit, A.err};
+        const int cap = 1 << A.nov_shift;
+        for (int r0 = 1; r0 <= ncand; r0 += 64) {
+            const int t = r0 + lane;
+            uint64_t v = 0;
+            bool novel = false;
+            if (t <= ncand) {
+                v = SM((int)(s_meta[t] & 0x3FFu));
+                novel = probe_table<false>(KP, phi_kmer_mix(v));
+            }
+            const unsigned long long ib = __ballot(novel);
+            const int pos = n_log + __popcll(ib & ((1ull << lane) - 1));
+            if (novel && pos < cap) A.nov_log[((A.log_base + chunk) << A.nov_shift) + pos] = v;
+            n_log += __popcll(ib);
+        }
+        n_emit = ncand;
+        if (n_log > cap) {
+            hashed = true;
+            n_log = 0; n_emit = 0;
+            if (lane == 0) s_meta[0] = (MetaT)ITEM_NOEMIT;
+            wave_sync();
+        }
+    }
diff --git a/phi_amd/csrc/sketch_win_fixed.hip b/phi_amd/csrc/sketch_win_fixed.hip
--- a/phi_amd/csrc/sketch_win_fixed.hip
+++ b/phi_amd/csrc/sketch_win_fixed.hip
@@ -76,6 +76,7 @@
         s_code[lane] = code;
         chunk_bad = __ballot(lane < 62 && bad != 0) != 0ull;
     }
+    const bool kmer_keys = !chunk_bad && A.k_rt != nullptr;
     wave_sync();
 
     {
@@ -159,14 +160,20 @@
                 }
             }
         }
-        if (coff == 0 && cflag) s_meta[0] = (MetaT)((uint32_t)(lane * Q + __ffs((int)cflag) - 2) | ITEM_NOEMIT);
+        if (coff == 0 && cflag && !kmer_keys) s_meta[0] = (MetaT)((uint32_t)(lane * Q + __ffs((int)cflag) - 2) | ITEM_NOEMIT);
     }
     wave_sync();
 #undef SQ
 
     int n_emit = 0, n_log = 0, n_nov_slow = 0;
     const int64_t out_base = 0;
+    bool hashed = !kmer_keys;
+    if (!hashed) {
+#include "sketch_rounds_kmer.inc"
+    }
+    if (hashed) {
 #include "sketch_rounds.inc"
+    }
 
     if (chunk_bad) {
         unsigned long long *s_bad_s = (unsigned long long *)(s_dyn + (size_t)__builtin_amdgcn_readfirstlane(wid) * phi_win_region_u64(R, s, w, k));
@@ -182,7 +189,7 @@
         if (PA->q_clean) clean_finish(*PA, chunk, (int64_t)gridDim.x * (TPB / 64), lane);
         if (lane == 0) {
             const int cap = 1 << PA->nov_shift;
-            PA->nov_cnt[PA->log_base + chunk] = (uint16_t)(n_log < cap ? n_log : cap);
+            PA->nov_cnt[PA->log_base + chunk] = (uint16_t)((uint32_t)(n_log < cap ? n_log : cap) | (hashed ? 0u : PHI_NOV_KMERS));
             const int n_nov_wave = n_log + n_nov_slow;
             const int stripe = (int)(chunk & (PHI_STRIPES - 1)) * 8;
             if (n_nov_wave && PA->n_logged) atomicAdd(PA->n_logged + stripe, (unsigned long long)n_nov_wave);
diff --git a/phi_amd/csrc/table.hip b/phi_amd/csrc/table.hip
--- a/phi_amd/csrc/table.hip
+++ b/phi_amd/csrc/table.hip
@@ -247,14 +247,45 @@
 __global__ void __launch_bounds__(256) phi_spectrum_flush_kernel(const uint64_t *__restrict__ nov_log, const uint16_t *__restrict__ nov_cnt,
                                                                  int64_t c_lo, int64_t n_ent, int32_t shift,
                                                                  uint64_t *__restrict__ sp_keys, uint64_t sp_mask,
-                                                                 unsigned long long *__restrict__ sp_count, uint32_t *__restrict__ err)
+                                                                 unsigned long long *__restrict__ sp_count, int32_t k,
+                                                                 const uint64_t *__restrict__ u_keys, uint64_t u_mask, uint32_t *__restrict__ err)
 {
     int n_new = 0;
-    for (int64_t t = (int64_t)blockIdx.x * blockDim.x + threadIdx.x; t < n_ent; t += (int64_t)gridDim.x * blockDim.x) {
-        const int64_t c = c_lo + (t >> shift);
-        const int i = (int)(t & ((1 << shift) - 1));
-        if (i >= (int)nov_cnt[c]) continue;
-        const uint64_t h = __builtin_nontemporal_load(&nov_log[(c << shift) + i]);
+    const int lane = threadIdx.x & 63;
+    for (int64_t t0 = (int64_t)blockIdx.x * blockDim.x + (threadIdx.x & ~63); t0 < n_ent; t0 += (int64_t)gridDim.x * blockDim.x) {
+        const int64_t t = t0 + lane;
+        bool have = false, kmers = false;
+        int i = 0;
+        int64_t c = 0;
+        uint64_t h = 0, v = 0;
+        if (t < n_ent) {
+            c = c_lo + (t >> shift);
+            i = (int)(t & ((1 << shift) - 1));
+            const uint32_t cnt = nov_cnt[c];
+            kmers = (cnt & PHI_NOV_KMERS) != 0;
+            have = i < (int)(cnt & (PHI_NOV_KMERS - 1));
+            if (have) {
+                h = __builtin_nontemporal_load(&nov_log[(c << shift) + i]);
+                if (kmers) { v = h; h = phi_kmer_hash(v, k); }
+            }
+        }
+        uint64_t hp = __shfl_up(h, 1, 64), vp = __shfl_up(v, 1, 64);
+        if (have && kmers) {
+            if (lane == 0 && i > 0) { vp = nov_log[(c << shift) + i - 1]; hp = phi_kmer_hash(vp, k); }
+            bool in_walks = false;
+            if (h != PHI_EMPTY_KEY) {
+                uint64_t su = h & u_mask;
+                for (int probes = 0; probes <= PHI_MAX_PROBE; probes++) {
+                    const uint64_t key = u_keys[su];
+                    if (key == h) { in_walks = true; break; }
+                    if (key == PHI_EMPTY_KEY) break;
+                    su = (su + 1) & u_mask;
+                }
+            }
+            const uint32_t e = phi_kmer_flush_rule(h, v, i > 0, hp, vp, in_walks);
+            if (e) { atomicOr(err, e); have = false; }
+        }
+        if (!have) continue;
         uint64_t slot = h & sp_mask;
         int probes = 0;
         for (;;) {
@@ -271,12 +302,60 @@
 }
 
 void phi_launch_spectrum_flush(hipStream_t st, const uint64_t *nov_log, const uint16_t *nov_cnt, int64_t c_lo, int64_t c_hi, int32_t shift,
-                               uint64_t *sp_keys, uint64_t sp_mask, unsigned long long *sp_count, uint32_t *err)
+                               uint64_t *sp_keys, uint64_t sp_mask, unsigned long long *sp_count, int32_t k, const uint64_t *u_keys,
+                               uint64_t u_mask, uint32_t *err)
 {
     const int64_t n_ent = (c_hi - c_lo) << shift;
     if (n_ent > 0)
         hipLaunchKernelGGL(phi_spectrum_flush_kernel, dim3(grid_for(n_ent, 256)), dim3(256), 0, st, nov_log, nov_cnt, c_lo, n_ent, shift,
-                           sp_keys, sp_mask, sp_count, err);
+                           sp_keys, sp_mask, sp_count, k, u_keys, u_mask, err);
+}
+
+__global__ void __launch_bounds__(256) phi_kmer_keys_kernel(const int32_t *__restrict__ rec_cls, const int32_t *__restrict__ rec_rel,
+                                                            const uint64_t *__restrict__ rec_hash, const uint32_t *__restrict__ rec_slot,
+                                                            int64_t n_rec, const int64_t *__restrict__ cls_base, const uint8_t *__restrict__ cls_left,
+                                                            const uint64_t *__restrict__ words, const uint32_t *__restrict__ badbits, int32_t k,
+                                                            uint64_t *__restrict__ kkeys, unsigned long long *__restrict__ ctr)
+{
+    for (int64_t i = (int64_t)blockIdx.x * blockDim.x + threadIdx.x; i < n_rec; i += (int64_t)gridDim.x * blockDim.x) {
+        const int32_t c = rec_cls[i];
+        const int64_t p = cls_base[c] + cls_left[c] + rec_rel[i];
+        const int64_t wi = p >> 5;
+        const int s = (int)(p & 31);
+        const uint64_t bad = (((uint64_t)badbits[wi + 1] << 32) | badbits[wi]) >> s;
+        if (bad & ((1ull << k) - 1)) { atomicAdd(&ctr[0], 1ull); continue; }
+        const uint64_t f = phi_extract64(words, p) >> (64 - 2 * k), r = phi_revcomp(f, k);
+        const uint64_t v = f < r ? f : r;
+        if (phi_kmer_hash(v, k) != rec_hash[i]) { atomicAdd(&ctr[1], 1ull); continue; }
+        const uint64_t key = phi_kmer_mix(v);
+        unsigned long long *slot = (unsigned long long *)&kkeys[rec_slot[i]];
+        unsigned long long prev = __builtin_nontemporal_load(slot);
+        if (prev == PHI_EMPTY_KEY) prev = atomicCAS(slot, PHI_EMPTY_KEY, key);
+        if (prev != PHI_EMPTY_KEY && prev != key) atomicAdd(&ctr[2], 1ull);
+    }
+}
+void phi_launch_kmer_keys(hipStream_t st, const int32_t *rec_cls, const int32_t *rec_rel, const uint64_t *rec_hash, const uint32_t *rec_slot,
+                          int64_t n_rec, const int64_t *cls_base, const uint8_t *cls_left, const uint64_t *words, const uint32_t *badbits,
+                          int32_t k, uint64_t *kkeys, unsigned long long *ctr)
+{
+    if (n_rec > 0)
+        hipLaunchKernelGGL(phi_kmer_keys_kernel, dim3(grid_for(n_rec, 256)), dim3(256), 0, st, rec_cls, rec_rel, rec_hash, rec_slot, n_rec,
+                           cls_base, cls_left, words, badbits, k, kkeys, ctr);
+}
+
+__global__ void __launch_bounds__(256) phi_rt_overflowed_kernel(const uint64_t *__restrict__ rt, int64_t n_buckets,
+                                                                unsigned long long *__restrict__ n_out)
+{
+    int cnt = 0;
+    for (int64_t b = (int64_t)blockIdx.x * blockDim.x + threadIdx.x; b < n_buckets; b += (int64_t)gridDim.x * blockDim.x)
+        cnt += (int)((rt[4 * b + 1] >> 32) & PHI_RT_OVERFLOWED);
+    cnt = phi_wave_sum(cnt);
+    if ((threadIdx.x & 63) == 0 && cnt) atomicAdd(n_out, (unsigned long long)cnt);
+}
+void phi_launch_rt_overflowed(hipStream_t st, const uint64_t *rt, int64_t n_buckets, unsigned long long *n_out)
+{
+    if (n_buckets > 0)
+        hipLaunchKernelGGL(phi_rt_overflowed_kernel, dim3(grid_for(n_buckets, 256)), dim3(256), 0, st, rt, n_buckets, n_out);
 }
 
 __global__ void __launch_bounds__(256) phi_count_flags_kernel(const uint8_t *__restrict__ flags, int64_t n,
```

After: 473.1, median of 6. +4.8%, better.
